# HuiGuanLab/DL-DKD

Hardware: NVIDIA B200
Metric: query-video pairs scored+ranked/sec (higher is better)
Workload: dtype bf16

## Files before the change

### dl-dkd_b200/_lib.py

```python
import ctypes
import os
from ctypes import c_char_p, c_float, c_int32, c_int64, c_void_p

_HERE = os.path.dirname(os.path.abspath(__file__))
LIB_PATH = os.path.join(_HERE, "libdkd_b200.so")

_P = c_void_p
_I = c_int32
_L = c_int64
_F = c_float

PROTOTYPES = {
    "dkd_version": [],
    "dkd_error_string": [_I],
    "dkd_normalize_rows": [_P, _L, _I, _F, _P, _P, _P, _L, _P],
    "dkd_downsample_clips": [_P, _P, _I, _I, _I, _I, _P, _P],
    "dkd_build_proposals": [_P, _I, _I, _I, _P, _P, _P, _P],
    "dkd_score_max_f32": [_P, _I, _P, _I, _I, _I, _P, _P, _P, _L, _P, _P, _P, _P],
    "dkd_row_planes_bytes": [_I, _I, _I],
    "dkd_pack_rows_tf32": [_P, _I, _I, _I, _P, _P],
    "dkd_score_max_exact": [_P, _I, _P, _I, _I, _I, _P, _P, _P, _L, _P, _P, _P],
    "dkd_clip_planes_bytes": [_I, _I],
    "dkd_pack_clips_tf32": [_P, _I, _I, _I, _P, _P],
    "dkd_clip_score_f32": [_P, _I, _P, _P, _I, _I, _I, _P, _P, _L, _P, _P, _P, _P, _P, _L, _P],
    "dkd_score_max_bf16": [_P, _I, _I, _P, _I, _I, _I, _P, _P, _P, _P, _L, _P, _F, _P],
    "dkd_score_max_f16": [_P, _I, _I, _P, _I, _I, _I, _P, _P, _P, _P, _L, _P, _F, _P],
    "dkd_score_max_bf16_lists": [_P, _I, _I, _P, _I, _I, _I, _P, _P, _P, _L, _F, _P, _P, _L, _I, _P],
    "dkd_clip_score_list": [_P, _I, _P, _P, _I, _I, _I, _P, _P, _L, _P, _P, _L, _P],
    "dkd_build_proposals_f16": [_P, _I, _I, _I, _P, _P, _P],
    "dkd_select_flagged": [_P, _I, _I, _L, _L, _P, _P, _P, _P, _P, _P],
    "dkd_select_pairs_csr": [_P, _I, _I, _L, _F, _L, _P, _P, _P, _P, _P],
    "dkd_key_clip_dots": [_P, _P, _I, _I, _I, _I, _P, _P],
    "dkd_frame_attn_table": [_P, _P, _P, _I, _I, _I, _I, _P, _P, _P],
    "dkd_frame_fuse": [_P, _P, _I, _P, _P, _I, _I, _I, _I, _L, _F, _F, _F, _I, _P, _P, _P],
    "dkd_fuse_scores": [_P, _P, _F, _F, _P, _L, _P],
    "dkd_topk": [_P, _I, _I, _L, _I, _I, _P, _P, _P],
    "dkd_select_topk": [_P, _I, _I, _L, _I, _I, _P, _P, _P],
    "dkd_merge_topk": [_P, _P, _I, _I, _I, _P, _P, _P],
    "dkd_rank_of_gt": [_P, _I, _I, _L, _P, _P, _P, _P],
    "dkd_candidates_to_csr": [_P, _I, _I, _I, _I, _P, _P, _P, _P, _P],
    "dkd_frame_fuse_csr": [_P, _P, _P, _P, _P, _P, _P, _I, _I, _I, _F, _F, _F, _I, _P, _L, _P],
    "dkd_scatter_fuse": [_P, _P, _F, _F, _P, _P, _I, _L, _P, _P],
    "dkd_sort_candidates": [_P, _P, _I, _I, _I, _P, _P, _P],
    "dkd_sort_candidates_payload": [_P, _P, _P, _I, _I, _I, _I, _P, _P, _P, _P],
    "dkd_merge_topk_payload": [_P, _P, _P, _I, _I, _I, _I, _P, _P, _P, _P],
    "dkd_frame_fuse_csr_detail": [_P, _P, _P, _P, _P, _P, _P, _I, _I, _I, _F, _F, _F, _I, _P, _L, _P, _I, _I, _P],
    "dkd_scatter_fuse_detail": [_P, _P, _F, _F, _P, _P, _P, _P, _I, _L, _P, _P, _I, _P],
    "dkd_weight_planes_bytes": [_I, _I],
    "dkd_pack_weight_tf32": [_P, _I, _I, _P, _P],
    "dkd_linear_exact": [_P, _L, _I, _P, _I, _P, _I, _P, _P, _L, _P],
    "dkd_row_stats": [_P, _L, _I, _F, _P, _P],
    "dkd_layernorm_rows": [_P, _L, _L, _I, _P, _P, _F, _P, _L, _P, _I, _P, _P],
    "dkd_mha_small": [_P, _L, _I, _I, _I, _P, _I, _I, _I, _I, _F, _P, _L, _P],
    "dkd_row_inv_norms": [_P, _L, _I, _F, _P, _P],
    "dkd_train_curve": [_P, _P, _P, _P, _I, _I, _I, _P, _P],
    "dkd_train_sim_fwd": [_P, _P, _P, _P, _P, _P, _I, _I, _I, _I, _P, _P, _P, _P, _P, _P],
    "dkd_train_sim_bwd": [_P, _P, _P, _P, _P, _P, _I, _I, _I, _I, _P, _P, _P, _P, _P, _P, _P, _P, _P, _P],
    "dkd_kl_curve_loss": [_P, _P, _P, _I, _I, _F, _P, _P, _P],
    "dkd_train_losses_workspace_floats": [_I, _I],
    "dkd_train_losses": [_P, _P, _P, _P, _P, _P, _I, _I, _F, _I, _F, _F, _P, _P, _P, _P, _P],
}
_RESTYPES = {"dkd_error_string": c_char_p, "dkd_clip_planes_bytes": c_int64, "dkd_row_planes_bytes": c_int64,
             "dkd_weight_planes_bytes": c_int64,
             "dkd_train_losses_workspace_floats": c_int64}

_lib = None


class DkdError(RuntimeError):
    pass


def load():
    global _lib
    if _lib is not None:
        return _lib
    if not os.path.exists(LIB_PATH):
        raise DkdError(
            f"{LIB_PATH} not found: build it with `python dl-dkd_b200/build.py` "
            "(nvcc, sm_100a). dkd_b200 has no CPU / PyTorch fallback for the scoring path.")
    lib = ctypes.CDLL(LIB_PATH)
    for name, argtypes in PROTOTYPES.items():
        fn = getattr(lib, name)
        fn.argtypes = argtypes
        fn.restype = _RESTYPES.get(name, c_int32)
    _lib = lib
    return lib


def check(code: int, what: str):
    if code != 0:
        msg = load().dkd_error_string(code)
        raise DkdError(f"{what} failed with code {code}: {msg.decode() if msg else '?'}")


KERNELS_PER_CALL = {"dkd_candidates_to_csr": 3, "dkd_select_pairs_csr": 3, "dkd_train_sim_bwd": 2, "dkd_train_losses": 3,
                    "dkd_train_losses_workspace_floats": 0}
_launches = 0
_timed_names = set()
_timed_events = {}


def reset_counters():
    global _launches
    _launches = 0


def launch_count() -> int:
    return _launches


def set_timed(names):
    global _timed_names, _timed_events
    _timed_names = set(names)
    _timed_events = {n: [] for n in _timed_names}


def timed_results():
    import torch
    torch.cuda.synchronize()
    return {n: [a.elapsed_time(b) for a, b in evs] for n, evs in _timed_events.items()}


def call(name: str, *args):
    global _launches
    lib = load()
    if name in _timed_names:
        import torch
        a, b = torch.cuda.Event(enable_timing=True), torch.cuda.Event(enable_timing=True)
        a.record()
        check(getattr(lib, name)(*args), name)
        b.record()
        _timed_events[name].append((a, b))
    else:
        check(getattr(lib, name)(*args), name)
    _launches += KERNELS_PER_CALL.get(name, 1)
```

### dl-dkd_b200/csrc/dkd_exact_umma.cu

```cuda
#include "dkd_umma.cuh"
#include "dkd_scan.cuh"

namespace dkd {

constexpr int kXRows = 128;
constexpr int kXKB = 32;
constexpr int kXScanWarps = 4;
constexpr int kXStageWarps = 8;
constexpr int kXStagers = 4 * 32;
constexpr int kXMmaWarp = kXScanWarps + kXStageWarps;
constexpr int kXLoadWarp = kXMmaWarp + 1;
constexpr int kXThreads = (kXLoadWarp + 1) * 32;
constexpr int kXMaxAStages = 7;
constexpr int kXBStages = 3;
constexpr uint32_t kXBPlane = 32 * 128;
constexpr int kXTmemCols = 512;
constexpr uint32_t kXRowPitch = 128;
constexpr uint32_t kXSlotBytes = 32 * kXRowPitch;
constexpr uint32_t kXScanScratch = 32 * kXRows * 4;

struct ExactParams {
  const float* q; int M;
  const float* planes; const float* scale;
  int Nv, T, D;
  int b_bufs;
  int R, Npad;
  const uint8_t* mask;
  float* out_max; int32_t* out_arg; int64_t ld_out;
  const int32_t* vid_ptr; const int32_t* vid_cnt; const int32_t* q_list; const int32_t* out_slot;
  unsigned wait_ns;
  int Nv_real, tile_chunks, tiles_per_chunk;
  int64_t list_stride;
  const int32_t* known_key;
  int64_t known_ld;
  const float2* row_ss;
  const float* bias;
  int relu, n_cols;
};
constexpr int kXGroup = 4;
#ifndef DKD_X_LIST_SCAN
#define DKD_X_LIST_SCAN 0
#endif
#ifndef DKD_X_KNOWN
#define DKD_X_KNOWN 1
#endif
#ifndef DKD_X_STREAM_B0
#define DKD_X_STREAM_B0 0
#endif
#ifndef DKD_X_RING0
#define DKD_X_RING0 5
#endif
constexpr bool kXStreamB0 = DKD_X_STREAM_B0 != 0;
constexpr int kXListScan = DKD_X_LIST_SCAN;
constexpr int kXKnown = DKD_X_KNOWN;
constexpr bool kXTwoPhaseList = kXListScan != 0 || kXKnown != 0;

struct __align__(8) ExactCtl {
  uint64_t a_full[kXMaxAStages], a_empty[kXMaxAStages];
  uint64_t b_full[kXBStages], b_empty[kXBStages];
  uint64_t tmem_full[2], tmem_empty[2];
  uint32_t tmem_base;
};

__device__ __forceinline__ void cp_async16(uint32_t dst, const void* src, uint32_t src_bytes) {
  asm volatile("cp.async.cg.shared.global [%0], [%1], 16, %2;" ::"r"(dst), "l"(src), "r"(src_bytes) : "memory");
}
__device__ __forceinline__ void cp_async_commit() { asm volatile("cp.async.commit_group;" ::: "memory"); }
template <int N>
__device__ __forceinline__ void cp_async_wait() { asm volatile("cp.async.wait_group %0;" ::"n"(N) : "memory"); }
__device__ __forceinline__ void bulk_load(void* dst, const void* src, uint32_t bytes, uint64_t* bar) {
  asm volatile("cp.async.bulk.shared::cluster.global.mbarrier::complete_tx::bytes [%0], [%1], %2, [%3];"
               ::"r"(smem_u32(dst)), "l"(src), "r"(bytes), "r"(smem_u32(bar)) : "memory");
}
__device__ __forceinline__ void fence_proxy_async() { asm volatile("fence.proxy.async.shared::cta;" ::: "memory"); }
__device__ __forceinline__ void split_tf32(float x, uint32_t& hi, uint32_t& lo) {
  hi = (__float_as_uint(x) + 0x1000u) & 0xffffe000u;
  lo = __float_as_uint(x - __uint_as_float(hi));
}

__device__ __forceinline__ void tmem_st_16x256b_x4(uint32_t taddr, const uint32_t* r) {
  asm volatile(
      "tcgen05.st.sync.aligned.16x256b.x4.b32 [%0], {%1,%2,%3,%4,%5,%6,%7,%8,%9,%10,%11,%12,%13,%14,%15,%16};"
      ::"r"(taddr), "r"(r[0]), "r"(r[1]), "r"(r[2]), "r"(r[3]), "r"(r[4]), "r"(r[5]), "r"(r[6]), "r"(r[7]),
        "r"(r[8]), "r"(r[9]), "r"(r[10]), "r"(r[11]), "r"(r[12]), "r"(r[13]), "r"(r[14]), "r"(r[15])
      : "memory");
}
__device__ __forceinline__ void tmem_st_wait() { asm volatile("tcgen05.wait::st.sync.aligned;" ::: "memory"); }

__device__ __forceinline__ void umma_tf32_ts(uint32_t tmem_d, uint32_t tmem_a, uint64_t bdesc, uint32_t idesc, uint32_t accum) {
  asm volatile(
      "{\n\t.reg .pred p;\n\t"
      "setp.ne.b32 p, %4, 0;\n\t"
      "tcgen05.mma.cta_group::1.kind::tf32 [%0], [%1], %2, %3, p;\n\t}"
      ::"r"(tmem_d), "r"(tmem_a), "l"(bdesc), "r"(idesc), "r"(accum)
      : "memory");
}
__host__ __device__ __forceinline__ uint32_t make_idesc_tf32(int n, int m) {
  return (1u << 4) | (2u << 7) | (2u << 10) | ((uint32_t)(n >> 3) << 17) | ((uint32_t)(m >> 4) << 24);
}

__device__ __forceinline__ uint32_t sw128_off(int r, int c) {
  return (uint32_t)((r >> 3) * 1024 + (r & 7) * 128 + ((c ^ (r & 7)) << 4));
}

__device__ __forceinline__ void video_range(const ExactParams& p, int n, int& e0, int& count) {
  if (p.vid_ptr) { e0 = p.vid_ptr[n]; count = p.vid_cnt ? p.vid_cnt[n] : p.vid_ptr[n + 1] - e0; }
  else if (p.list_stride > 0) {
    e0 = (int)((int64_t)n * p.list_stride);
    count = p.vid_cnt[n];
    if (count > (int)p.list_stride) count = (int)p.list_stride;
  }
  else { e0 = 0; count = p.M; }
}

__device__ __forceinline__ void item_range(const ExactParams& p, int item, int& group, int& row0, int& count) {
  group = item / p.tile_chunks;
  const int chunk = item - group * p.tile_chunks;
  row0 = chunk * p.tiles_per_chunk * kXRows;
  const int rows = p.tiles_per_chunk * kXRows;
  count = p.M - row0 < rows ? p.M - row0 : rows;
}

__device__ __forceinline__ void item_range_linear(const ExactParams& p, int item, int& wtile, int& row0, int& count) {
  wtile = item % p.Nv_real;
  const int chunk = item / p.Nv_real;
  row0 = chunk * p.tiles_per_chunk * kXRows;
  const int rows = p.tiles_per_chunk * kXRows;
  count = p.M - row0 < rows ? p.M - row0 : rows;
}

template <int kMode, bool kT32, int kXRing>
__global__ void __launch_bounds__(kXThreads, 1)
exact_umma_kernel(const ExactParams p) {
  constexpr int kDW = kMode == 0 ? 32 : 128;
  constexpr int kScaleBufs = kMode == 2 ? kXGroup : 2;
  constexpr int kStageSets = kMode == 2 ? 1 : 2;
  constexpr int kScanGroups = (kMode == 0 && kXTwoPhaseList) ? 1 : 0;
  constexpr bool kResB = kMode == 0 && !kXStreamB0;
  constexpr uint32_t kXACol0 = 2 * kDW;
  constexpr int kXStages = (kXTmemCols - 2 * kDW) / 64;
  extern __shared__ __align__(1024) uint8_t smem_raw_x[];
  __shared__ __align__(16) float s_scale[kScaleBufs][32 * 32];
  uint8_t* smem = reinterpret_cast<uint8_t*>((reinterpret_cast<uintptr_t>(smem_raw_x) + 1023) & ~(uintptr_t)1023);
  const int num_kb = p.D / kXKB;
  const uint32_t b_buf_bytes = kResB ? (uint32_t)num_kb * 2u * kXBPlane : 2u * (uint32_t)p.Npad * 128u;
  uint8_t* sB = smem;
  uint8_t* sS = sB + (size_t)(kResB ? p.b_bufs : kXBStages) * b_buf_bytes;
  float* sD = reinterpret_cast<float*>(sS + (size_t)(4 * kStageSets) * kXRing * kXSlotBytes);
  ExactCtl* ctl = reinterpret_cast<ExactCtl*>(reinterpret_cast<uint8_t*>(sD) + (size_t)kScanGroups * kXScanScratch);
  const int warp = threadIdx.x >> 5, lane = threadIdx.x & 31;
  const uint32_t b_bufs = (uint32_t)p.b_bufs;

  if (threadIdx.x == 0) {
    for (int i = 0; i < kXStages; ++i) { mbar_init(&ctl->a_full[i], kXStagers); mbar_init(&ctl->a_empty[i], 1); }
    for (int i = 0; i < kXBStages; ++i) { mbar_init(&ctl->b_full[i], 1); mbar_init(&ctl->b_empty[i], 1); }
    for (int i = 0; i < 2; ++i) {
      mbar_init(&ctl->tmem_full[i], 1);
      mbar_init(&ctl->tmem_empty[i], kXScanWarps);
    }
    fence_barrier_init();
  }
  if (warp == kXMmaWarp) {
    asm volatile("tcgen05.alloc.cta_group::1.sync.aligned.shared::cta.b32 [%0], %1;" ::"r"(smem_u32(&ctl->tmem_base)), "n"(kXTmemCols));
    asm volatile("tcgen05.relinquish_alloc_permit.cta_group::1.sync.aligned;");
  }
  tc_fence_before();
  __syncthreads();
  tc_fence_after();
  const uint32_t tmem_base = ctl->tmem_base;

  if (warp >= kXScanWarps && warp < kXScanWarps + 4 * kStageSets) {
    const int quarter = warp & 3, par = (warp - kXScanWarps) >> 2;
    const int g = lane >> 2, t = lane & 3;
    const int cl_row = lane >> 3, cl_chunk = lane & 7;
    const uint32_t a_lane = tmem_base + ((uint32_t)(quarter * 32) << 16) + kXACol0;
    const int sw = warp - kXScanWarps;
    const uint32_t ring0 = smem_u32(sS) + (uint32_t)sw * kXRing * kXSlotBytes;
    const uint8_t* ring_ptr = sS + (size_t)sw * kXRing * kXSlotBytes;
    uint32_t it_base = 0;
    for (int n = blockIdx.x; n < p.Nv; n += gridDim.x) {
      int e0, count, row_base = 0;
      if (kMode == 2) { int g_; item_range(p, n, g_, row_base, count); e0 = 0; }
      else if (kMode == 4) { int g_; item_range_linear(p, n, g_, row_base, count); e0 = 0; }
      else video_range(p, n, e0, count);
      if (count <= 0) continue;
      int ss_tile = -1;
      float2 ss[4];
      const int nitems = ((count + kXRows - 1) / kXRows) * num_kb;
      int t_cached = -1;
      const float* src_cached[8];
      uint32_t live_mask = 0;
      int iss_tile = 0, iss_kb = par;
      while (iss_kb >= num_kb) { iss_kb -= num_kb; ++iss_tile; }
      auto issue = [&](int slot) {
        const int tile = iss_tile, kb = iss_kb;
        iss_kb += kStageSets;
        while (iss_kb >= num_kb) { iss_kb -= num_kb; ++iss_tile; }
        if (tile != t_cached) {
          t_cached = tile;
          live_mask = 0;
#pragma unroll
          for (int i = 0; i < 8; ++i) {
            const int r = tile * kXRows + quarter * 32 + 4 * i + cl_row;
            const bool live = r < count;
            const int64_t qrow = live ? (p.q_list ? (int64_t)p.q_list[e0 + r] : (int64_t)(row_base + r)) : 0;
            src_cached[i] = p.q + qrow * p.D + 4 * cl_chunk;
            live_mask |= (live ? 1u : 0u) << i;
          }
        }
        const uint32_t dst = ring0 + (uint32_t)slot * kXSlotBytes + (uint32_t)cl_row * kXRowPitch +
                             (uint32_t)((cl_chunk ^ ((cl_row & 1) << 2)) << 4);
#pragma unroll
        for (int i = 0; i < 8; ++i)
          cp_async16(dst + (uint32_t)(4 * i) * kXRowPitch, src_cached[i] + kb * kXKB, ((live_mask >> i) & 1u) ? 16u : 0u);
      };
      auto store = [&](int j, int slot_i) {
        const uint8_t* slot = ring_ptr + (size_t)slot_i * kXSlotBytes;
        float4 v[8];
#pragma unroll
        for (int hu = 0; hu < 4; ++hu)
#pragma unroll
          for (int c = 0; c < 2; ++c)
            v[2 * hu + c] = *reinterpret_cast<const float4*>(
                slot + (16 * (hu >> 1) + g + 8 * (hu & 1)) * kXRowPitch + (((4 * c + t) ^ ((g & 1) << 2)) << 4));
        if (kMode == 4) {
          if (p.row_ss) {
            const int tile_j = j / num_kb;
            if (tile_j != ss_tile) {
              ss_tile = tile_j;
#pragma unroll
              for (int hu = 0; hu < 4; ++hu) {
                const int r = tile_j * kXRows + quarter * 32 + 16 * (hu >> 1) + g + 8 * (hu & 1);
                ss[hu] = r < count ? __ldg(p.row_ss + row_base + r) : make_float2(0.f, 0.f);
              }
            }
#pragma unroll
            for (int hu = 0; hu < 4; ++hu)
#pragma unroll
              for (int c = 0; c < 2; ++c) {
                float4& x = v[2 * hu + c];
                x.x = fmaf(x.x, ss[hu].x, ss[hu].y); x.y = fmaf(x.y, ss[hu].x, ss[hu].y);
                x.z = fmaf(x.z, ss[hu].x, ss[hu].y); x.w = fmaf(x.w, ss[hu].x, ss[hu].y);
              }
          }
        }
        const uint32_t it = it_base + (uint32_t)j;
        const uint32_t stage = it % (uint32_t)kXStages;
        const uint32_t phase = (it / (uint32_t)kXStages) & 1u;
        mbar_wait_backoff(&ctl->a_empty[stage], phase ^ 1u, 5 * p.wait_ns);
        tc_fence_after();
#pragma unroll
        for (int h = 0; h < 2; ++h) {
          uint32_t rh[16], rl[16];
#pragma unroll
          for (int u = 0; u < 2; ++u)
#pragma unroll
            for (int c = 0; c < 2; ++c) {
              const float4 x = v[2 * (2 * h + u) + c];
              split_tf32(x.x, rh[4 * (2 * c) + 2 * u + 0], rl[4 * (2 * c) + 2 * u + 0]);
              split_tf32(x.y, rh[4 * (2 * c) + 2 * u + 1], rl[4 * (2 * c) + 2 * u + 1]);
              split_tf32(x.z, rh[4 * (2 * c + 1) + 2 * u + 0], rl[4 * (2 * c + 1) + 2 * u + 0]);
              split_tf32(x.w, rh[4 * (2 * c + 1) + 2 * u + 1], rl[4 * (2 * c + 1) + 2 * u + 1]);
            }
          const uint32_t ta = a_lane + ((uint32_t)(16 * h) << 16) + stage * 64u;
          tmem_st_16x256b_x4(ta, rh);
          tmem_st_16x256b_x4(ta + 32u, rl);
        }
        tmem_st_wait();
        tc_fence_before();
        mbar_arrive(&ctl->a_full[stage]);
      };
      const int nmine = (nitems - par + kStageSets - 1) / kStageSets;
#pragma unroll
      for (int m = 0; m < kXRing - 1; ++m) {
        if (m < nmine) issue(m);
        cp_async_commit();
      }
      for (int m = 0; m < nmine; ++m) {
        if (m + kXRing - 1 < nmine) issue((m + kXRing - 1) % kXRing);
        cp_async_commit();
        cp_async_wait<kXRing - 1>();
        __syncwarp();
        store(kStageSets * m + par, m % kXRing);
        __syncwarp();
      }
      cp_async_wait<0>();
      it_base += (uint32_t)nitems;
    }
  } else if (warp == kXLoadWarp) {
    if (lane == 0) {
      uint32_t vi = 0, itb = 0;
      for (int n = blockIdx.x; n < p.Nv; n += gridDim.x) {
        int e0, count;
        if (kMode == 2) {
          int g_, row0_;
          item_range(p, n, g_, row0_, count);
          if (count <= 0) continue;
          const uint8_t* base = reinterpret_cast<const uint8_t*>(p.planes);
          for (int t0 = 0; t0 < count; t0 += kXRows) {
            for (int kb = 0; kb < num_kb; ++kb, ++itb) {
              const uint32_t bs = itb % (uint32_t)kXBStages;
              mbar_wait_backoff(&ctl->b_empty[bs], ((itb / (uint32_t)kXBStages) & 1u) ^ 1u, 5 * p.wait_ns);
              mbar_expect_tx(&ctl->b_full[bs], b_buf_bytes);
              for (int v = 0; v < kXGroup; ++v) {
                const int vid = min(g_ * kXGroup + v, p.Nv_real - 1);
                const uint8_t* src = base + ((size_t)vid * num_kb + kb) * 2 * kXBPlane;
                bulk_load(sB + (size_t)bs * b_buf_bytes + (size_t)v * kXBPlane, src, kXBPlane, &ctl->b_full[bs]);
                bulk_load(sB + (size_t)bs * b_buf_bytes + (size_t)(kXGroup + v) * kXBPlane, src + kXBPlane, kXBPlane,
                          &ctl->b_full[bs]);
              }
            }
          }
          continue;
        }
        int vid = n;
        if (kMode == 4) { int r0_; item_range_linear(p, n, vid, r0_, count); }
        else video_range(p, n, e0, count);
        if (count <= 0) continue;
        if (kResB) {
          const uint32_t bb = vi % b_bufs;
          mbar_wait_backoff(&ctl->b_empty[bb], ((vi / b_bufs) & 1u) ^ 1u, 5 * p.wait_ns);
          ++vi;
          mbar_expect_tx(&ctl->b_full[bb], b_buf_bytes);
          const uint8_t* src = reinterpret_cast<const uint8_t*>(p.planes) + (size_t)n * b_buf_bytes;
          for (int kb = 0; kb < num_kb; ++kb)
            bulk_load(sB + (size_t)bb * b_buf_bytes + (size_t)kb * 2 * kXBPlane, src + (size_t)kb * 2 * kXBPlane,
                      2 * kXBPlane, &ctl->b_full[bb]);
        } else {
          const uint8_t* src = reinterpret_cast<const uint8_t*>(p.planes) + (size_t)vid * num_kb * b_buf_bytes;
          for (int t0 = 0; t0 < count; t0 += kXRows) {
            for (int kb = 0; kb < num_kb; ++kb, ++itb) {
              const uint32_t bs = itb % (uint32_t)kXBStages;
              mbar_wait_backoff(&ctl->b_empty[bs], ((itb / (uint32_t)kXBStages) & 1u) ^ 1u, 5 * p.wait_ns);
              mbar_expect_tx(&ctl->b_full[bs], b_buf_bytes);
              bulk_load(sB + (size_t)bs * b_buf_bytes, src + (size_t)kb * b_buf_bytes, b_buf_bytes, &ctl->b_full[bs]);
            }
          }
        }
      }
    }
  } else if (warp == kXMmaWarp) {
    const int nb = kMode == 0 ? 32 : p.Npad;
    const uint32_t idesc = make_idesc_tf32(nb, kXRows);
    const uint32_t b_plane = (uint32_t)nb * 128u;
    const bool elected = elect_one();
    const uint64_t bdesc0 = make_smem_desc(smem_u32(sB));
    uint32_t it = 0, vi = 0, tc = 0, itb = 0;
    for (int n = blockIdx.x; n < p.Nv; n += gridDim.x) {
      int e0, count;
      if (kMode == 2) { int g_, r_; item_range(p, n, g_, r_, count); e0 = 0; }
      else if (kMode == 4) { int g_, r_; item_range_linear(p, n, g_, r_, count); e0 = 0; }
      else video_range(p, n, e0, count);
      if (count <= 0) continue;
      uint32_t bb = 0;
      if (kResB) {
        bb = vi % b_bufs;
        mbar_wait_backoff(&ctl->b_full[bb], (vi / b_bufs) & 1u, p.wait_ns);
        ++vi;
      }
      for (int t0 = 0; t0 < count; t0 += kXRows, ++tc) {
        const uint32_t buf = tc & 1u;
        mbar_wait_backoff(&ctl->tmem_empty[buf], ((tc >> 1) & 1u) ^ 1u, p.wait_ns);
        tc_fence_after();
        const uint32_t d_tmem = tmem_base + buf * (uint32_t)kDW;
        for (int kb = 0; kb < num_kb; ++kb, ++it) {
          const uint32_t stage = it % (uint32_t)kXStages;
          const uint32_t phase = (it / (uint32_t)kXStages) & 1u;
          uint32_t bs = 0;
          if (!kResB) {
            bs = itb % (uint32_t)kXBStages;
            mbar_wait_backoff(&ctl->b_full[bs], (itb / (uint32_t)kXBStages) & 1u, p.wait_ns);
            ++itb;
          }
          mbar_wait_backoff(&ctl->a_full[stage], phase, p.wait_ns);
          tc_fence_after();
          if (elected) {
            const uint32_t a_hi = tmem_base + kXACol0 + stage * 64u;
            const uint32_t a_lo = a_hi + 32u;
            const uint64_t b_hi = kResB ? bdesc0 + (uint64_t)((bb * b_buf_bytes + (uint32_t)kb * 2u * b_plane) >> 4)
                                             : bdesc0 + (uint64_t)((bs * b_buf_bytes) >> 4);
            const uint64_t b_lo = b_hi + (uint64_t)(b_plane >> 4);
#pragma unroll
            for (int k = 0; k < 4; ++k) {
              umma_tf32_ts(d_tmem, a_lo + 8 * k, b_hi + 2 * k, idesc, (kb | k) ? 1u : 0u);
              umma_tf32_ts(d_tmem, a_hi + 8 * k, b_lo + 2 * k, idesc, 1u);
              umma_tf32_ts(d_tmem, a_hi + 8 * k, b_hi + 2 * k, idesc, 1u);
            }
            umma_commit(&ctl->a_empty[stage]);
            if (!kResB) umma_commit(&ctl->b_empty[bs]);
          }
          __syncwarp();
        }
        if (elected) umma_commit(&ctl->tmem_full[buf]);
        __syncwarp();
      }
      if (kResB) {
        if (elected) umma_commit(&ctl->b_empty[bb]);
        __syncwarp();
      }
    }
  } else if constexpr (kMode == 2) {
    const int T = p.T, P = T * (T + 1) / 2;
    const int quarter = warp & 3;
    const uint32_t part = warp >= 2 * kXScanWarps ? 1u : 0u;
    const int stid = threadIdx.x;
    uint32_t tc = 0;
    for (int n = blockIdx.x; n < p.Nv; n += gridDim.x) {
      int group, row0, count;
      item_range(p, n, group, row0, count);
      if (count <= 0) continue;
      asm volatile("bar.sync 1, %0;" ::"n"(2 * kXScanWarps * 32) : "memory");
      if (part == 0) {
        for (int v = 0; v < kXGroup; ++v) {
          const int vid = min(group * kXGroup + v, p.Nv_real - 1);
          const float* gsc = p.scale + (int64_t)vid * P;
          const int s_ = stid & 31;
          int base = 0;
          for (int w = 1; w <= T; ++w) {
            if ((w & 3) == (stid >> 5) && s_ + w <= T) s_scale[v][(w - 1) * 32 + s_] = __ldg(gsc + base + s_);
            base += T - w + 1;
          }
        }
      }
      asm volatile("bar.sync 1, %0;" ::"n"(2 * kXScanWarps * 32) : "memory");
      for (int t0 = 0; t0 < count; t0 += kXRows, ++tc) {
        const uint32_t buf = tc & 1u;
        if (buf != part) continue;
        mbar_wait(&ctl->tmem_full[buf], (tc >> 1) & 1u);
        tc_fence_after();
        const int r = row0 + t0 + quarter * 32 + lane;
#pragma unroll 1
        for (int v = 0; v < kXGroup; ++v) {
          uint32_t raw[32];
          tmem_ld32_issue(tmem_base + ((uint32_t)(quarter * 32) << 16) + buf * (uint32_t)kDW + (uint32_t)(32 * v), raw);
          tmem_ld_wait();
          if (v == kXGroup - 1) {
            tc_fence_before();
            __syncwarp();
            if (lane == 0) mbar_arrive(&ctl->tmem_empty[buf]);
          }
          const float* sc = s_scale[v];
          float d[32];
#pragma unroll
          for (int i = 0; i < 32; ++i) d[i] = __uint_as_float(raw[i]);
          float bv0;
          int bi0;
          window_scan_v1<kT32>(d, sc, T, bv0, bi0);
          const int vid = group * kXGroup + v;
          if (r < p.M && t0 + quarter * 32 + lane < count && vid < p.Nv_real) {
            const int64_t o = (int64_t)r * p.ld_out + vid;
            p.out_max[o] = bv0;
            if (p.out_arg) p.out_arg[o] = bi0;
          }
        }
      }
    }
  } else if constexpr (kMode == 0) {
    const int T = p.T, P = T * (T + 1) / 2;
    const int quarter = warp;
    const int stid = threadIdx.x;
    uint32_t tc = 0, vi = 0;
    for (int n = blockIdx.x; n < p.Nv; n += gridDim.x) {
      int e0, count;
      video_range(p, n, e0, count);
      if (count <= 0) continue;
      float* sc = s_scale[vi & 1u];
      {
        const float* gsc = p.scale + (int64_t)n * P;
        const int s_ = stid & 31;
        int base = 0;
        for (int w = 1; w <= T; ++w) {
          if ((w & 3) == (stid >> 5) && s_ + w <= T) sc[(w - 1) * 32 + s_] = __ldg(gsc + base + s_);
          base += T - w + 1;
        }
      }
      asm volatile("bar.sync 1, %0;" ::"n"(kXScanWarps * 32) : "memory");
      ++vi;
      for (int t0 = 0; t0 < count; t0 += kXRows, ++tc) {
        const uint32_t buf = tc & 1u;
        mbar_wait(&ctl->tmem_full[buf], (tc >> 1) & 1u);
        tc_fence_after();
        uint32_t raw[32];
        tmem_ld32_issue(tmem_base + ((uint32_t)(quarter * 32) << 16) + buf * (uint32_t)kDW, raw);
        tmem_ld_wait();
        tc_fence_before();
        __syncwarp();
        if (lane == 0) mbar_arrive(&ctl->tmem_empty[buf]);
        float d[32];
#pragma unroll
        for (int i = 0; i < 32; ++i) d[i] = __uint_as_float(raw[i]);
        float bv0;
        int bi0;
        const int r = t0 + quarter * 32 + lane;
        if constexpr (kT32 && kXTwoPhaseList) {
          float* dcol = sD + quarter * 32 + lane;
          if (kXKnown != 0 && p.known_key) {
            const int qi = r < count ? (p.q_list ? p.q_list[e0 + r] : r) : 0;
            const int key = r < count ? __ldg(p.known_key + (int64_t)qi * p.known_ld + n) : 0;
            window_scan_known<kXKnown == 2>(d, sc, dcol, kXRows, key, bv0, bi0);
          } else if (kXListScan != 0) {
            window_scan_v2<kXListScan == 2>(d, sc, dcol, kXRows, bv0, bi0);
          } else {
            window_scan_v1<kT32>(d, sc, T, bv0, bi0);
          }
        } else {
          window_scan_v1<kT32>(d, sc, T, bv0, bi0);
        }
        if (r < count) {
          const int64_t o = p.out_slot ? (int64_t)p.out_slot[e0 + r]
                            : (p.list_stride > 0 ? (int64_t)p.q_list[e0 + r] * p.ld_out + n
                                                 : (p.vid_ptr ? (int64_t)(e0 + r) : (int64_t)r * p.ld_out + n));
          p.out_max[o] = bv0;
          if (p.out_arg) p.out_arg[o] = bi0;
        }
      }
    }
  } else if constexpr (kMode == 4) {
    const int quarter = warp;
    uint32_t tc = 0;
    for (int n = blockIdx.x; n < p.Nv; n += gridDim.x) {
      int wtile, row0, count;
      item_range_linear(p, n, wtile, row0, count);
      if (count <= 0) continue;
      for (int t0 = 0; t0 < count; t0 += kXRows, ++tc) {
        const uint32_t buf = tc & 1u;
        mbar_wait(&ctl->tmem_full[buf], (tc >> 1) & 1u);
        tc_fence_after();
        const int r = t0 + quarter * 32 + lane;
        const bool live = r < count;
        float* orow = p.out_max + (int64_t)(row0 + (live ? r : 0)) * p.ld_out;
#pragma unroll 1
        for (int c0 = 0; c0 < 128; c0 += 32) {
          uint32_t raw[32];
          tmem_ld32_issue(tmem_base + ((uint32_t)(quarter * 32) << 16) + buf * (uint32_t)kDW + (uint32_t)c0, raw);
          tmem_ld_wait();
          if (c0 == 96) {
            tc_fence_before();
            __syncwarp();
            if (lane == 0) mbar_arrive(&ctl->tmem_empty[buf]);
          }
#pragma unroll
          for (int j = 0; j < 32; j += 4) {
            const int col = wtile * 128 + c0 + j;
            if (live && col < p.n_cols) {
              float4 o = make_float4(__uint_as_float(raw[j]), __uint_as_float(raw[j + 1]), __uint_as_float(raw[j + 2]),
                                     __uint_as_float(raw[j + 3]));
              if (p.bias) {
                const float4 b = __ldg(reinterpret_cast<const float4*>(p.bias + col));
                o.x += b.x; o.y += b.y; o.z += b.z; o.w += b.w;
              }
              if (p.relu) { o.x = fmaxf(o.x, 0.f); o.y = fmaxf(o.y, 0.f); o.z = fmaxf(o.z, 0.f); o.w = fmaxf(o.w, 0.f); }
              *reinterpret_cast<float4*>(orow + col) = o;
            }
          }
        }
      }
    }
  } else {
    const int quarter = warp;
    uint32_t tc = 0;
    for (int n = blockIdx.x; n < p.Nv; n += gridDim.x) {
      int e0, count;
      video_range(p, n, e0, count);
      if (count <= 0) continue;
      const uint8_t* mrow = p.mask ? p.mask + (int64_t)n * p.R : nullptr;
      for (int t0 = 0; t0 < count; t0 += kXRows, ++tc) {
        const uint32_t buf = tc & 1u;
        mbar_wait(&ctl->tmem_full[buf], (tc >> 1) & 1u);
        tc_fence_after();
        float bv = -INFINITY;
        int bi = 0;
        for (int c0 = 0; c0 < p.R; c0 += 32) {
          uint32_t raw[32];
          tmem_ld32_issue(tmem_base + ((uint32_t)(quarter * 32) << 16) + buf * (uint32_t)kDW + (uint32_t)c0, raw);
          tmem_ld_wait();
#pragma unroll
          for (int j = 0; j < 32; ++j) {
            const int r = c0 + j;
            if (r < p.R) {
              float v = __uint_as_float(raw[j]);
              if (mrow && __ldg(mrow + r) == 0) v = DKD_MASKED_SCORE;
              if (v > bv) { bv = v; bi = r; }
            }
          }
        }
        tc_fence_before();
        __syncwarp();
        if (lane == 0) mbar_arrive(&ctl->tmem_empty[buf]);
        const int r = t0 + quarter * 32 + lane;
        if (r < count) {
          const int64_t o = p.out_slot ? (int64_t)p.out_slot[e0 + r]
                                       : (p.vid_ptr ? (int64_t)(e0 + r) : (int64_t)r * p.ld_out + n);
          p.out_max[o] = bv;
          if (p.out_arg) p.out_arg[o] = bi;
        }
      }
    }
  }

  tc_fence_before();
  __syncthreads();
  if (warp == kXMmaWarp) {
    tc_fence_after();
    asm volatile("tcgen05.dealloc.cta_group::1.sync.aligned.b32 %0, %1;" ::"r"(tmem_base), "n"(kXTmemCols));
  }
}

__global__ void pack_rows_tf32_kernel(const float* __restrict__ x, int R, int rpad, int D, float* __restrict__ planes,
                                      int64_t total_rows) {
  const int n = blockIdx.x;
  const int num_kb = D / kXKB;
  const uint32_t plane_bytes = (uint32_t)rpad * 128u;
  uint8_t* dst = reinterpret_cast<uint8_t*>(planes) + (size_t)n * num_kb * 2 * plane_bytes;
  for (int i = threadIdx.x; i < num_kb * rpad * 8; i += blockDim.x) {
    const int kb = i / (rpad * 8), rem = i - kb * rpad * 8;
    const int r = rem >> 3, c8 = rem & 7;
    float4 v = make_float4(0.f, 0.f, 0.f, 0.f);
    if (r < R && (int64_t)n * R + r < total_rows) v = *reinterpret_cast<const float4*>(x + ((int64_t)n * R + r) * D + kb * kXKB + c8 * 4);
    uint2 h0, l0, h1, l1;
    split_tf32(v.x, h0.x, l0.x); split_tf32(v.y, h0.y, l0.y); split_tf32(v.z, h1.x, l1.x); split_tf32(v.w, h1.y, l1.y);
    const int cc = c8 >> 2, tt = c8 & 3;
    const int p0 = 16 * cc + 2 * tt;
    uint8_t* row0 = dst + (size_t)(kb * 2) * plane_bytes;
    uint8_t* d0 = row0 + sw128_off(r, p0 >> 2) + (p0 & 3) * 4;
    uint8_t* d1 = row0 + sw128_off(r, (p0 + 8) >> 2) + (p0 & 3) * 4;
    *reinterpret_cast<uint2*>(d0) = h0;
    *reinterpret_cast<uint2*>(d1) = h1;
    *reinterpret_cast<uint2*>(d0 + plane_bytes) = l0;
    *reinterpret_cast<uint2*>(d1 + plane_bytes) = l1;
  }
}

}

using namespace dkd;

static int row_pad(int R, int clip_mode) { return clip_mode ? 32 : ((R + 15) / 16) * 16; }

extern "C" int64_t dkd_clip_planes_bytes(int32_t Nv, int32_t D) {
  if (Nv < 0 || D <= 0 || D % kXKB != 0) return -1;
  return (int64_t)Nv * (D / kXKB) * 2 * kXBPlane;
}
extern "C" int64_t dkd_row_planes_bytes(int32_t Nv, int32_t R, int32_t D) {
  if (Nv < 0 || R <= 0 || R > 128 || D <= 0 || D % kXKB != 0) return -1;
  return (int64_t)Nv * (D / kXKB) * 2 * row_pad(R, 0) * 128;
}

static int pack_rows(const float* x, int32_t Nv, int32_t R, int32_t rpad, int32_t D, float* planes, void* stream) {
  if (!x || !planes || Nv < 0) return DKD_ERR_ARG;
  if (R <= 0 || R > rpad || D <= 0 || D % kXKB != 0 || D > 512) return DKD_ERR_SHAPE;
  if ((reinterpret_cast<uintptr_t>(x) | reinterpret_cast<uintptr_t>(planes)) & 15) return DKD_ERR_ALIGN;
  if (Nv == 0) return DKD_OK;
  pack_rows_tf32_kernel<<<Nv, 256, 0, (cudaStream_t)stream>>>(x, R, rpad, D, planes, (int64_t)Nv * R);
  DKD_LAUNCH_CHECK();
  return DKD_OK;
}
extern "C" int dkd_pack_clips_tf32(const float* clips, int32_t Nv, int32_t T, int32_t D, float* planes, void* stream) {
  if (T > 32) return DKD_ERR_SHAPE;
  return pack_rows(clips, Nv, T, 32, D, planes, stream);
}
extern "C" int dkd_pack_rows_tf32(const float* xn, int32_t Nv, int32_t R, int32_t D, float* planes, void* stream) {
  if (R > 128) return DKD_ERR_SHAPE;
  return pack_rows(xn, Nv, R, row_pad(R, 0), D, planes, stream);
}

static int launch_exact(int mode, ExactParams p, int32_t D, int32_t T, cudaStream_t st) {
  p.wait_ns = 0u;
  int dev = 0, sms = 0, max_smem = 0;
  DKD_CUDA_TRY(cudaGetDevice(&dev));
  DKD_CUDA_TRY(cudaDeviceGetAttribute(&sms, cudaDevAttrMultiProcessorCount, dev));
  DKD_CUDA_TRY(cudaDeviceGetAttribute(&max_smem, cudaDevAttrMaxSharedMemoryPerBlockOptin, dev));
  const int num_kb = D / kXKB;
  const bool stream0 = mode == 0 && kXStreamB0;
  const int ring = stream0 ? DKD_X_RING0 : ((mode == 0 || mode == 2) && D > 448 ? 2 : 3);
  const int ring_warps = mode == 2 ? 4 : kXStageWarps;
  const int scan_groups = (mode == 0 && kXTwoPhaseList) ? 1 : 0;
  const size_t fixed = sizeof(ExactCtl) + 1024 + 128 + 16384  +
                       (size_t)ring_warps * ring * kXSlotBytes + (size_t)scan_groups * kXScanScratch;
  size_t b_total;
  if (mode == 0 && !stream0) {
    const size_t b_buf = (size_t)num_kb * 2 * kXBPlane;
    if ((size_t)max_smem < fixed + b_buf) return DKD_ERR_SHAPE;
    p.b_bufs = ((size_t)max_smem >= fixed + 2 * b_buf) ? 2 : 1;
    b_total = (size_t)p.b_bufs * b_buf;
  } else {
    p.b_bufs = kXBStages;
    b_total = (size_t)kXBStages * 2 * p.Npad * 128;
    if ((size_t)max_smem < fixed + b_total) return DKD_ERR_SHAPE;
  }
  const size_t smem = fixed - 16384 + b_total;
  const int grid = p.Nv < sms ? p.Nv : sms;
  auto launch = [&](auto kern) -> int {
    DKD_CUDA_TRY(cudaFuncSetAttribute(kern, cudaFuncAttributeMaxDynamicSharedMemorySize, (int)smem));
    kern<<<grid, kXThreads, smem, st>>>(p);
    return DKD_OK;
  };
  int rc;
  if (mode == 0 && stream0) {
    rc = (T == 32) ? launch(exact_umma_kernel<0, true, DKD_X_RING0>) : launch(exact_umma_kernel<0, false, DKD_X_RING0>);
  } else if (mode == 0) {
    if (ring == 3) rc = (T == 32) ? launch(exact_umma_kernel<0, true, 3>) : launch(exact_umma_kernel<0, false, 3>);
    else rc = (T == 32) ? launch(exact_umma_kernel<0, true, 2>) : launch(exact_umma_kernel<0, false, 2>);
  } else if (mode == 2) {
    if (ring == 3) rc = (T == 32) ? launch(exact_umma_kernel<2, true, 3>) : launch(exact_umma_kernel<2, false, 3>);
    else rc = (T == 32) ? launch(exact_umma_kernel<2, true, 2>) : launch(exact_umma_kernel<2, false, 2>);
  } else if (mode == 4) {
    rc = launch(exact_umma_kernel<4, true, 3>);
  } else {
    rc = launch(exact_umma_kernel<1, true, 3>);
  }
  if (rc) return rc;
  DKD_LAUNCH_CHECK();
  return DKD_OK;
}

extern "C" int dkd_score_max_exact(const float* qn, int32_t M, const float* row_planes, int32_t Nv, int32_t R,
                                   int32_t D, const uint8_t* mask, float* out_max, int32_t* out_arg,
                                   int64_t ld_out, const int32_t* vid_ptr, const int32_t* q_list, void* stream) {
  if (!qn || !row_planes || !out_max || M < 0 || Nv < 0) return DKD_ERR_ARG;
  if ((vid_ptr == nullptr) != (q_list == nullptr)) return DKD_ERR_ARG;
  if (R <= 0 || R > 128 || D <= 0 || D % kXKB != 0 || D > 512) return DKD_ERR_SHAPE;
  if (!vid_ptr && ld_out < Nv) return DKD_ERR_ARG;
  if ((reinterpret_cast<uintptr_t>(qn) | reinterpret_cast<uintptr_t>(row_planes)) & 15) return DKD_ERR_ALIGN;
  if (M == 0 || Nv == 0) return DKD_OK;
  ExactParams p{};
  p.q = qn; p.M = M; p.planes = row_planes; p.scale = nullptr;
  p.Nv = Nv; p.T = 0; p.D = D; p.R = R; p.Npad = row_pad(R, 0); p.mask = mask;
  p.out_max = out_max; p.out_arg = out_arg; p.ld_out = ld_out;
  p.vid_ptr = vid_ptr; p.vid_cnt = nullptr; p.q_list = q_list; p.out_slot = nullptr;
  return launch_exact(1, p, D, 0, (cudaStream_t)stream);
}

extern "C" int dkd_clip_score_f32(const float* qn, int32_t M, const float* clip_planes, const float* prop_scale,
                                  int32_t Nv, int32_t T, int32_t D, float* out_max, int32_t* out_arg,
                                  int64_t ld_out, const int32_t* vid_ptr, const int32_t* vid_cnt,
                                  const int32_t* q_list, const int32_t* out_slot, const int32_t* known_key,
                                  int64_t known_ld, void* stream) {
  if (!qn || !clip_planes || !prop_scale || !out_max || M < 0 || Nv < 0) return DKD_ERR_ARG;
  if ((vid_ptr == nullptr) != (q_list == nullptr)) return DKD_ERR_ARG;
  if ((out_slot || vid_cnt) && !vid_ptr) return DKD_ERR_ARG;
  if (known_key && (!vid_ptr || known_ld < Nv || T != 32)) return DKD_ERR_ARG;
  if (T <= 0 || T > 32 || D <= 0 || D % kXKB != 0 || D > 512) return DKD_ERR_SHAPE;
  if (!vid_ptr && ld_out < Nv) return DKD_ERR_ARG;
  if ((reinterpret_cast<uintptr_t>(qn) | reinterpret_cast<uintptr_t>(clip_planes) | reinterpret_cast<uintptr_t>(prop_scale)) & 15)
    return DKD_ERR_ALIGN;
  if (M == 0 || Nv == 0) return DKD_OK;
  ExactParams p{};
  p.q = qn; p.M = M; p.planes = clip_planes; p.scale = prop_scale;
  p.Nv = Nv; p.T = T; p.D = D; p.R = T; p.Npad = 32; p.mask = nullptr;
  p.out_max = out_max; p.out_arg = out_arg; p.ld_out = ld_out;
  p.vid_ptr = vid_ptr; p.vid_cnt = vid_cnt; p.q_list = q_list; p.out_slot = out_slot;
  p.known_key = known_key; p.known_ld = known_ld;
  if (!vid_ptr && Nv >= kXGroup) {
    const int groups = (Nv + kXGroup - 1) / kXGroup;
    const int tiles = (M + kXRows - 1) / kXRows;
    int sms = 148, dev = 0;
    if (cudaGetDevice(&dev) == cudaSuccess) cudaDeviceGetAttribute(&sms, cudaDevAttrMultiProcessorCount, dev);
    int chunks = 1;
    while (chunks < tiles && (int64_t)groups * chunks < (int64_t)sms * 12) ++chunks;
    p.tiles_per_chunk = (tiles + chunks - 1) / chunks;
    p.tile_chunks = (tiles + p.tiles_per_chunk - 1) / p.tiles_per_chunk;
    p.Nv_real = Nv;
    p.Nv = groups * p.tile_chunks;
    p.Npad = 128;
    return launch_exact(2, p, D, T, (cudaStream_t)stream);
  }
  return launch_exact(0, p, D, T, (cudaStream_t)stream);
}

extern "C" int64_t dkd_weight_planes_bytes(int32_t N, int32_t K) {
  if (N <= 0 || K <= 0 || K % kXKB != 0) return -1;
  return (int64_t)((N + 127) / 128) * (K / kXKB) * 2 * 128 * 128;
}

extern "C" int dkd_pack_weight_tf32(const float* w, int32_t N, int32_t K, float* planes, void* stream) {
  if (!w || !planes || N <= 0) return DKD_ERR_ARG;
  if (K <= 0 || K % kXKB != 0) return DKD_ERR_SHAPE;
  if ((reinterpret_cast<uintptr_t>(w) | reinterpret_cast<uintptr_t>(planes)) & 15) return DKD_ERR_ALIGN;
  pack_rows_tf32_kernel<<<(N + 127) / 128, 256, 0, (cudaStream_t)stream>>>(w, 128, 128, K, planes, (int64_t)N);
  DKD_LAUNCH_CHECK();
  return DKD_OK;
}

extern "C" int dkd_linear_exact(const float* x, int64_t M, int32_t K, const float* w_planes, int32_t N,
                                const float* bias, int32_t relu, const float* row_scale_shift, float* out,
                                int64_t ld_out, void* stream) {
  if (!x || !w_planes || !out || M < 0 || N <= 0) return DKD_ERR_ARG;
  if (K <= 0 || K % kXKB != 0 || N % 4 != 0 || ld_out < N || ld_out % 4 != 0 || M > 0x7fffff00LL) return DKD_ERR_SHAPE;
  if ((reinterpret_cast<uintptr_t>(x) | reinterpret_cast<uintptr_t>(w_planes) | reinterpret_cast<uintptr_t>(out) |
       reinterpret_cast<uintptr_t>(bias) | reinterpret_cast<uintptr_t>(row_scale_shift)) & 15)
    return DKD_ERR_ALIGN;
  if (M == 0) return DKD_OK;
  ExactParams p{};
  p.q = x; p.M = (int)M; p.planes = w_planes; p.scale = nullptr;
  p.T = 0; p.D = K; p.R = 128; p.Npad = 128; p.mask = nullptr;
  p.out_max = out; p.out_arg = nullptr; p.ld_out = ld_out;
  p.row_ss = reinterpret_cast<const float2*>(row_scale_shift); p.bias = bias; p.relu = relu; p.n_cols = N;
  const int wtiles = (N + 127) / 128;
  const int tiles = (int)((M + kXRows - 1) / kXRows);
  int sms = 148, dev = 0;
  if (cudaGetDevice(&dev) == cudaSuccess) cudaDeviceGetAttribute(&sms, cudaDevAttrMultiProcessorCount, dev);
  int chunks = 1;
  while (chunks < tiles && (int64_t)wtiles * chunks < (int64_t)sms * 6) ++chunks;
  p.tiles_per_chunk = (tiles + chunks - 1) / chunks;
  p.tile_chunks = (tiles + p.tiles_per_chunk - 1) / p.tiles_per_chunk;
  p.Nv_real = wtiles;
  p.Nv = wtiles * p.tile_chunks;
  return launch_exact(4, p, K, 0, (cudaStream_t)stream);
}

extern "C" int dkd_clip_score_list(const float* qn, int32_t M, const float* clip_planes, const float* prop_scale,
                                   int32_t Nv, int32_t T, int32_t D, float* out_max, int32_t* out_arg, int64_t ld_out,
                                   const int32_t* vid_cnt, const int32_t* q_list, int64_t list_stride, void* stream) {
  if (!qn || !clip_planes || !prop_scale || !out_max || !vid_cnt || !q_list || M < 0 || Nv < 0) return DKD_ERR_ARG;
  if (list_stride <= 0 || ld_out < Nv || (int64_t)Nv * list_stride > 0x7fffffffLL) return DKD_ERR_ARG;
  if (T <= 0 || T > 32 || D <= 0 || D % kXKB != 0 || D > 512) return DKD_ERR_SHAPE;
  if ((reinterpret_cast<uintptr_t>(qn) | reinterpret_cast<uintptr_t>(clip_planes) | reinterpret_cast<uintptr_t>(prop_scale)) & 15)
    return DKD_ERR_ALIGN;
  if (M == 0 || Nv == 0) return DKD_OK;
  ExactParams p{};
  p.q = qn; p.M = M; p.planes = clip_planes; p.scale = prop_scale;
  p.Nv = Nv; p.T = T; p.D = D; p.R = T; p.Npad = 32; p.mask = nullptr;
  p.out_max = out_max; p.out_arg = out_arg; p.ld_out = ld_out;
  p.vid_ptr = nullptr; p.vid_cnt = vid_cnt; p.q_list = q_list; p.out_slot = nullptr; p.list_stride = list_stride;
  return launch_exact(0, p, D, T, (cudaStream_t)stream);
}
```

### dl-dkd_b200/engine.py

```python
import math
from dataclasses import dataclass, field
from typing import List, Optional

import torch
import torch.nn.functional as F

from . import ops

BRANCH_WEIGHTS = (0.7, 0.3)


@dataclass
class BranchData:
    frames_n: Optional[torch.Tensor] = None
    frames_b: Optional[torch.Tensor] = None
    frame_planes: Optional[torch.Tensor] = None
    clips: Optional[torch.Tensor] = None
    clip_planes: Optional[torch.Tensor] = None
    prop_scale: Optional[torch.Tensor] = None
    prop_b: Optional[torch.Tensor] = None
    prop_h: Optional[torch.Tensor] = None
    frames_h: Optional[torch.Tensor] = None
    table_f: Optional[torch.Tensor] = None
    table_h: Optional[torch.Tensor] = None


@dataclass
class PreparedCorpus:
    Nv: int
    L: int
    D: int
    T: int
    id_base: int
    mask_u8: torch.Tensor
    lengths: torch.Tensor
    branches: List[BranchData] = field(default_factory=list)
    heads: tuple = ("frame", "two_scale")
    Lg: int = 0
    mask_g: Optional[torch.Tensor] = None
    Pg: int = 0
    prop_mask: Optional[torch.Tensor] = None

    @property
    def P(self):
        return ops.num_proposals(self.T)

    def nbytes(self):
        tot = 0
        for b in self.branches:
            for t in vars(b).values():
                if t is not None:
                    tot += t.numel() * t.element_size()
        return tot


def prepare_corpus(frames_by_branch, mask, attn_params=None, T=ops.T_CLIPS, heads=("frame", "two_scale"),
                   precisions=("exact", "bf16"), id_base=0) -> PreparedCorpus:
    f0 = frames_by_branch[0]
    Nv, L, D = f0.shape
    mask = mask.to(f0.device)
    mask_u8 = (mask > 0).to(torch.uint8).contiguous()
    lengths = mask_u8.sum(dim=1).to(torch.int32).contiguous()
    pc = PreparedCorpus(Nv=Nv, L=L, D=D, T=T, id_base=id_base, mask_u8=mask_u8, lengths=lengths, heads=tuple(heads))
    P = ops.num_proposals(T)
    pc.Lg, pc.Pg = ops.round_up(L, 16), ops.round_up(P, 16)
    pc.mask_g = mask_u8
    if pc.Lg != L:
        pc.mask_g = torch.zeros((Nv, pc.Lg), dtype=torch.uint8, device=f0.device)
        pc.mask_g[:, :L] = mask_u8
    if pc.Pg != P:
        pc.prop_mask = torch.zeros((Nv, pc.Pg), dtype=torch.uint8, device=f0.device)
        pc.prop_mask[:, :P] = 1
    if Nv == 0:
        pc.branches = [BranchData() for _ in frames_by_branch]
        return pc

    def pad_rows(t, R, Rg):
        if t is None or Rg == R:
            return t
        out = torch.zeros((Nv, Rg, D), dtype=t.dtype, device=t.device)
        out[:, :R] = t.view(Nv, R, D)
        return out.view(Nv * Rg, D)

    for bi, fr in enumerate(frames_by_branch):
        fr = fr.contiguous().float()
        bd = BranchData()
        if "frame" in heads:
            approx = "bf16" in precisions or "fp16" in precisions
            out = ops.normalize_rows(fr, want_f32="exact" in precisions or approx,
                                     want_bf16="bf16" in precisions, want_f16="fp16" in precisions)
            fn, fb, fh = out if len(out) == 3 else (out[0], out[1], None)
            bd.frames_n = None if fn is None else fn.view(Nv, L, D)
            bd.frames_b = pad_rows(fb, L, pc.Lg)
            bd.frames_h = pad_rows(fh, L, pc.Lg)
            if bd.frames_n is not None and D % 32 == 0:
                bd.frame_planes = ops.pack_rows(bd.frames_n)
        if "two_scale" in heads:
            if attn_params is None:
                raise ValueError("two_scale head needs the key/value projections (attn_params)")
            kw, kb, vw, vb = attn_params[bi]
            bd.clips = ops.downsample_clips(fr, lengths, T)
            bd.clip_planes = ops.pack_clips(bd.clips)
            pb, ps, _ = ops.build_proposals(bd.clips, want_bf16="bf16" in precisions, want_scale=True)
            bd.prop_b = None if pb is None else pad_rows(pb.view(-1, D), P, pc.Pg)
            bd.prop_scale = ps
            if "fp16" in precisions:
                bd.prop_h = pad_rows(ops.build_proposals_f16(bd.clips)[0].view(-1, D), P, pc.Pg)
            key = F.linear(fr, kw, kb).contiguous()
            val = F.linear(fr, vw, vb).contiguous()
            bd.table_f, bd.table_h = ops.frame_attn_table(key, val, bd.clips, lengths, want_f32=True,
                                                          want_f16=any(x in precisions for x in ("bf16", "fp16", "shortcut")))
            del key, val
        pc.branches.append(bd)
    return pc


@dataclass
class PreparedQueries:
    M: int
    Mpad: int
    qn: List[torch.Tensor]
    qb: List[torch.Tensor]
    qh: List[torch.Tensor]


_PAD_WORDS = {}


@dataclass
class HitDetail:
    arg: torch.Tensor
    score: torch.Tensor
    frame: Optional[torch.Tensor] = None

    @staticmethod
    def pad_words(nb, two_scale, device=None):
        key = (nb, bool(two_scale), str(device))
        if key not in _PAD_WORDS:
            ninf = torch.tensor([float("-inf")], dtype=torch.float32).view(torch.int32).item()
            _PAD_WORDS[key] = torch.tensor(([-1, ninf, ninf] if two_scale else [-1, ninf]) * nb, dtype=torch.int32,
                                           device=device)
        return _PAD_WORDS[key]

    @classmethod
    def padding(cls, M, K, nb, two_scale, device=None):
        return cls.unpack(cls.pad_words(nb, two_scale, device).expand(M, K, -1), nb, two_scale)

    def pack(self) -> torch.Tensor:
        M, K, nb = self.arg.shape
        parts = [self.arg, self.score.view(torch.int32)]
        if self.frame is not None:
            parts.append(self.frame.view(torch.int32))
        return torch.stack(parts, dim=-1).reshape(M, K, nb * len(parts))

    @classmethod
    def unpack(cls, words, nb, two_scale):
        M, K, _ = words.shape
        w = words.reshape(M, K, nb, 3 if two_scale else 2)
        return cls(arg=w[..., 0].contiguous(), score=w[..., 1].contiguous().view(torch.float32),
                   frame=w[..., 2].contiguous().view(torch.float32) if two_scale else None)

    @classmethod
    def cat(cls, details):
        return cls(arg=torch.cat([d.arg for d in details]), score=torch.cat([d.score for d in details]),
                   frame=None if details[0].frame is None else torch.cat([d.frame for d in details]))

    def patch(self, idx, other):
        self.arg[idx] = other.arg
        self.score[idx] = other.score
        if self.frame is not None:
            self.frame[idx] = other.frame


def _gather_detail(ids, id_base, args, scores, frames=None):
    valid = (ids >= 0).unsqueeze(-1)
    n = (ids.long() - id_base).clamp_(min=0)

    def take(mats, fill):
        out = torch.stack([m.gather(1, n) for m in mats], dim=-1)
        return out.masked_fill_(~valid, fill)

    return HitDetail(arg=take(args, -1), score=take(scores, float("-inf")),
                     frame=None if frames is None else take(frames, float("-inf")))


def prepare_queries(q_by_branch, want_bf16=True) -> PreparedQueries:
    M = q_by_branch[0].shape[0]
    Mpad = ops.round_up(max(M, 1), 256)
    qn, qb, qh = [], [], []
    if M == 0:
        return PreparedQueries(M=0, Mpad=Mpad, qn=[q.float() for q in q_by_branch], qb=[None] * len(q_by_branch),
                               qh=[None] * len(q_by_branch))
    for q in q_by_branch:
        f, b, h = ops.normalize_rows(q.contiguous().float(), want_f32=True, want_bf16=want_bf16, rows_pad=Mpad,
                                     want_f16=True)
        qn.append(f[:M])
        qb.append(b)
        qh.append(h)
    return PreparedQueries(M=M, Mpad=Mpad, qn=qn, qb=qb, qh=qh)


def _branch_weights(nb):
    return BRANCH_WEIGHTS[:nb] if nb == 2 else (1.0,)


def _exact_rows(bd: BranchData, qn, pc: PreparedCorpus, csr=None):
    if bd.frame_planes is not None:
        return ops.score_max_exact(qn, bd.frame_planes, pc.L, pc.mask_u8, csr=csr)
    s, a, _ = ops.score_max_f32(qn, bd.frames_n, pc.mask_u8, csr=csr)
    return s, a


def score_frame_head(pc: PreparedCorpus, pq: PreparedQueries, precision="exact", want_arg=False):
    out = []
    for bd, qn, qb, qh in zip(pc.branches, pq.qn, pq.qb, pq.qh):
        if precision == "exact":
            s, a = _exact_rows(bd, qn, pc)
        elif precision == "fp16":
            s, a = ops.score_max_bf16(qh, pq.M, bd.frames_h, pc.Nv, pc.Lg, pc.mask_g)
        else:
            s, a = ops.score_max_bf16(qb, pq.M, bd.frames_b, pc.Nv, pc.Lg, pc.mask_g)
        out.append((s, a))
    return out


AMBIGUITY_TAU = 1.0e-3
AMBIGUITY_TAU_F16 = AMBIGUITY_TAU / 8


def score_two_scale_head(pc: PreparedCorpus, pq: PreparedQueries, precision="exact", w_clip=0.7, w_frame=0.3,
                         want_frame=False, tau=None):
    nb = len(pc.branches)
    wbs = _branch_weights(nb)
    fused = None
    per = []
    if tau is None:
        tau = AMBIGUITY_TAU_F16 if precision == "fp16" else AMBIGUITY_TAU
    for bi, (bd, qn, qb, qh) in enumerate(zip(pc.branches, pq.qn, pq.qb, pq.qh)):
        if precision == "exact":
            s_clip, k_clip = ops.clip_score_f32(qn, bd.clip_planes, bd.prop_scale)
            q, tab = qn, bd.table_f
        elif precision == "shortcut":
            s_clip, k_clip = ops.clip_score_f32(qn, bd.clip_planes, bd.prop_scale)
            q, tab = qh, bd.table_h
        else:
            if precision == "fp16":
                qb, prop = qh, bd.prop_h
            else:
                prop = bd.prop_b
            if tau > 0:
                s_clip, k_clip, cnt, lst = ops.score_max_bf16_lists(qb, pq.M, prop, pc.Nv, pc.Pg, tau, mask=pc.prop_mask)
                ops.clip_score_list(qn, bd.clip_planes, bd.prop_scale, cnt, lst, s_clip, k_clip)
            else:
                s_clip, k_clip = ops.score_max_bf16(qb, pq.M, prop, pc.Nv, pc.Pg, mask=pc.prop_mask)
            q, tab = qh, bd.table_h
        wb = wbs[bi] if nb == 2 else 1.0
        fused, fr = ops.frame_fuse(q, tab, s_clip, k_clip, w_clip, w_frame, wb, fused=fused, accumulate=bi > 0,
                                   want_frame=want_frame)
        per.append(dict(clip=s_clip, key_clip=k_clip, frame=fr))
    return fused, per


CERT_EPS = 1.0e-3
CERT_EPS_F16 = 2.5e-4
STATS = {"certify_fallback_queries": 0, "certify_checked_queries": 0}


class PendingCertificate:

    def __init__(self, pc, pq, unsure, out_s, out_i, args, detail=None):
        self.pc, self.pq, self.unsure, self.out_s, self.out_i, self.args = pc, pq, unsure, out_s, out_i, args
        self.detail = detail
        self.host = torch.empty((1,), dtype=torch.int32).pin_memory()
        self.host.copy_(unsure.sum(dtype=torch.int32).reshape(1), non_blocking=True)
        self.event = torch.cuda.Event()
        self.event.record()

    def resolve(self):
        self.event.synchronize()
        return _apply_fallback(self.pc, self.pq, self.unsure, int(self.host[0]), self.out_s, self.out_i, self.args,
                               self.detail)


PENDING: List[PendingCertificate] = []


def finish(keep_last=0):
    n = 0
    while len(PENDING) > keep_last:
        n += PENDING.pop(0).resolve()
    return n


def poll():
    n = 0
    while PENDING and PENDING[0].event.query():
        n += PENDING.pop(0).resolve()
    return n


def _apply_fallback(pc, pq, unsure, n_unsure, out_s, out_i, args, detail=None):
    STATS["certify_checked_queries"] += pq.M
    STATS["certify_fallback_queries"] += n_unsure
    if n_unsure:
        nb = len(pc.branches)
        idx = unsure.nonzero().squeeze(1)
        sub = PreparedQueries(M=n_unsure, Mpad=ops.round_up(n_unsure, 256), qn=[q[idx].contiguous() for q in pq.qn],
                              qb=[None] * nb, qh=[None] * nb)
        if detail is None:
            es, ei = rank(pc, sub, precision="exact", **args)
        else:
            es, ei, ed = rank(pc, sub, precision="exact", return_detail=True, **args)
            detail.patch(idx, ed)
        out_s[idx] = es
        out_i[idx] = ei
    return n_unsure


def rank(pc: PreparedCorpus, pq: PreparedQueries, K=100, head="two_scale", precision="bf16", rescore=True,
         Kc=128, w_clip=0.7, w_frame=0.3, tau=None, certify=True, return_dense=False, return_detail=False):
    nb = len(pc.branches)
    wbs = _branch_weights(nb)
    two = head != "frame"
    if PENDING:
        poll()
    if pq.M == 0 or pc.Nv == 0:
        dev = pc.mask_u8.device
        out = (torch.full((pq.M, K), float("-inf"), dtype=torch.float32, device=dev),
               torch.full((pq.M, K), -1, dtype=torch.int32, device=dev))
        if return_dense:
            out += (torch.empty((pq.M, pc.Nv), dtype=torch.float32, device=dev),)
        return out + (HitDetail.padding(pq.M, K, nb, two, dev),) if return_detail else out
    dense_route = precision == "exact" or not rescore
    per = None
    if head == "frame":
        if precision == "shortcut":
            raise ValueError("precision='shortcut' is a two-scale variant (the frame head has no clip windows)")
        sc = score_frame_head(pc, pq, precision)
        fused = sc[0][0] if nb == 1 else ops.fuse_scores(sc[0][0], sc[1][0], wbs[0], wbs[1])
    else:
        fused, per = score_two_scale_head(pc, pq, precision, w_clip, w_frame, tau=tau,
                                          want_frame=return_detail and dense_route)
    extra = (fused,) if return_dense else ()
    if dense_route:
        out_s, out_i = ops.topk(fused, K, pc.id_base)
        if return_detail:
            if head == "frame":
                det = _gather_detail(out_i, pc.id_base, [a for _, a in sc], [s for s, _ in sc])
            else:
                det = _gather_detail(out_i, pc.id_base, [p["key_clip"] for p in per], [p["clip"] for p in per],
                                     [p["frame"] for p in per])
            extra += (det,)
        return (out_s, out_i) + extra
    Kc = max(Kc, K)
    cand, approx_kth = ops.select_topk(fused, Kc, pc.id_base)
    csr = ops.candidates_to_csr(cand, pc.Nv, pc.id_base)
    cand_scores = torch.full((pq.M, Kc), float("-inf"), dtype=torch.float32, device=cand.device)
    words = torch.empty((pq.M, Kc, nb * (3 if two else 2)), dtype=torch.int32, device=cand.device) if return_detail \
        else None
    if head == "frame":
        ex = [_exact_rows(bd, qn, pc, csr=csr[:2]) for bd, qn in zip(pc.branches, pq.qn)]
        if return_detail:
            b, ab = (ex[1][0], ex[1][1]) if nb == 2 else (None, None)
            ops.scatter_fuse_detail(ex[0][0], b, wbs[0], wbs[1] if nb == 2 else 0.0, ex[0][1], ab, csr, cand_scores,
                                    words)
        elif nb == 2:
            ops.scatter_fuse(ex[0][0], ex[1][0], wbs[0], wbs[1], csr, cand_scores)
        else:
            ops.scatter_fuse(ex[0][0], None, 1.0, 0.0, csr, cand_scores)
    else:
        for bi, (bd, qn) in enumerate(zip(pc.branches, pq.qn)):
            if precision == "shortcut":
                cs, ck = per[bi]["clip"], per[bi]["key_clip"]
            else:
                cs, ck = ops.clip_score_f32(qn, bd.clip_planes, bd.prop_scale, csr=csr[:2],
                                            known_key=per[bi]["key_clip"])
            wb = wbs[bi] if nb == 2 else 1.0
            if return_detail:
                ops.frame_fuse_csr_detail(qn, bd.table_f, cs, ck, csr, w_clip, w_frame, wb, cand_scores, bi > 0,
                                          words, 3 * bi)
            else:
                ops.frame_fuse_csr(qn, bd.table_f, cs, ck, csr, w_clip, w_frame, wb, cand_scores, bi > 0)
    detail = None
    if return_detail:
        out_s, out_i, out_w = ops.sort_candidates_payload(cand_scores, cand, words, K,
                                                          HitDetail.pad_words(nb, two, cand.device))
        detail = HitDetail.unpack(out_w, nb, two)
    else:
        out_s, out_i = ops.sort_candidates(cand_scores, cand, K)
    if certify and Kc < pc.Nv:
        unsure = out_s[:, K - 1] <= approx_kth + (CERT_EPS if precision == "bf16" else CERT_EPS_F16)
        args = dict(K=K, head=head, w_clip=w_clip, w_frame=w_frame)
        if certify == "deferred":
            PENDING.append(PendingCertificate(pc, pq, unsure, out_s, out_i, args, detail))
        else:
            _apply_fallback(pc, pq, unsure, int(unsure.sum()), out_s, out_i, args, detail)
    return (out_s, out_i) + extra + ((detail,) if return_detail else ())


def moment_frames(arg, ids, lengths, T=ops.T_CLIPS, head="two_scale"):
    valid = (ids >= 0).unsqueeze(-1) & (arg >= 0)
    if head == "frame":
        first, end = arg.long(), arg.long() + 1
    else:
        P = ops.num_proposals(T)
        ws = torch.tensor([ops.proposal_window(p, T) for p in range(P)], dtype=torch.long, device=arg.device)
        p = arg.long().clamp(0, P - 1)
        w, s = ws[p, 0], ws[p, 1]
        n = torch.as_tensor(lengths, device=arg.device)[ids.long().clamp(min=0)].unsqueeze(-1).expand_as(arg)
        nf, nl = n.float(), n.long()

        def a(i):
            return torch.minimum(torch.round(i.float() / T * nf).long(), nl - 1)

        first, end = a(s), torch.maximum(a(s + w), a(s + w - 1) + 1)
    out = torch.stack([first, end], dim=-1).to(torch.int32)
    return out.masked_fill_(~valid.unsqueeze(-1), -1)


def shard_range(Nv: int, rank_: int, world: int):
    per = (Nv + world - 1) // world
    lo = min(rank_ * per, Nv)
    return lo, min(lo + per, Nv)


def _merge_lists(scores, ids, words=None, pad=None):
    if words is None:
        return ops.merge_topk(scores, ids)
    return ops.merge_topk_payload(scores, ids, words, pad)


def merge_shards(local_scores, local_ids, group=None, merge_fn=None, exchange="query_block", gather=True, detail=None):
    import torch.distributed as dist
    world = dist.get_world_size(group)
    M, K = local_scores.shape
    if detail is None:
        merge = merge_fn or ops.merge_topk
        local = [local_scores.contiguous(), local_ids.contiguous()]
        finish = tuple
    else:
        nb, two = detail.arg.shape[-1], detail.frame is not None
        pad = HitDetail.pad_words(nb, two, local_scores.device)
        merge = merge_fn or (lambda s, i, w: _merge_lists(s, i, w, pad))
        local = [local_scores.contiguous(), local_ids.contiguous(), detail.pack()]

        def finish(res):
            return (res[0], res[1], HitDetail.unpack(res[2], nb, two))
    if world == 1:
        res = finish(local)
        return res if gather else res[:2] + ((0, M),) + res[2:]
    dev = local_scores.device
    nccl = dist.get_backend(group) == "nccl"
    if exchange == "all_gather":
        gathered = [torch.empty((world,) + t.shape, dtype=t.dtype, device=dev) for t in local]
        for g, t in zip(gathered, local):
            if nccl:
                dist.all_gather_into_tensor(g, t, group=group)
            else:
                dist.all_gather(list(g.unbind(0)), t, group=group)
        res = finish(merge(*gathered))
        return res if gather else res[:2] + ((0, M),) + res[2:]
    if exchange != "query_block":
        raise ValueError("exchange must be 'query_block' or 'all_gather'")
    rank_ = dist.get_rank(group)
    Mb = (M + world - 1) // world
    q_lo, q_hi = min(rank_ * Mb, M), min((rank_ + 1) * Mb, M)
    mine = q_hi - q_lo
    in_split = [min((g + 1) * Mb, M) - min(g * Mb, M) for g in range(world)]
    recv = [torch.empty((world, mine) + t.shape[1:], dtype=t.dtype, device=dev) for t in local]
    for r, t in zip(recv, local):
        row = math.prod(t.shape[1:])
        dist.all_to_all_single(r.view(world * mine, row), t.view(M, row), [mine] * world, in_split, group=group)
    if mine:
        block = list(merge(*recv))
    else:
        block = [r.new_empty((0,) + r.shape[2:]) for r in recv]
    if not gather:
        res = finish(block)
        return res[:2] + ((q_lo, q_hi),) + res[2:]
    if mine != Mb:
        fills = [float("-inf"), -1, -1]
        block = [torch.cat([b, b.new_full((Mb - mine,) + b.shape[1:], f)]) for b, f in zip(block, fills)]
    full = [torch.empty((world * Mb,) + b.shape[1:], dtype=b.dtype, device=dev) for b in block]
    for f, b in zip(full, block):
        if nccl:
            dist.all_gather_into_tensor(f, b.contiguous(), group=group)
        else:
            dist.all_gather(list(f.view((world, Mb) + b.shape[1:]).unbind(0)), b.contiguous(), group=group)
    return finish([f[:M] for f in full])


def split_queries(q_by_branch, batch=16384):
    Nq = q_by_branch[0].shape[0]
    return [prepare_queries([q[lo: lo + batch] for q in q_by_branch]) for lo in range(0, max(Nq, 1), batch)]


def iter_chunks(frames_by_branch, mask, chunk_videos=8192, id_base=0):
    Nv = frames_by_branch[0].shape[0]
    for lo in range(0, Nv, chunk_videos):
        hi = min(lo + chunk_videos, Nv)
        yield [f[lo:hi] for f in frames_by_branch], mask[lo:hi], id_base + lo


def rank_streamed(chunks, pqs, attn_params=None, K=100, T=ops.T_CLIPS, head="two_scale", precision="bf16",
                  rescore=True, Kc=128, w_clip=0.7, w_frame=0.3, tau=None, return_detail=False):
    running = [None] * len(pqs)
    precisions = ("exact", precision) if precision != "exact" else ("exact",)
    for frames, mask, id_base in chunks:
        pc = prepare_corpus(frames, mask, attn_params, T=T, heads=(head,), precisions=precisions, id_base=id_base)
        for b, pq in enumerate(pqs):
            out = rank(pc, pq, K=K, head=head, precision=precision, rescore=rescore, Kc=Kc, w_clip=w_clip,
                       w_frame=w_frame, tau=tau, return_detail=return_detail)
            if running[b] is None:
                running[b] = out
            elif not return_detail:
                running[b] = ops.merge_topk(torch.stack([running[b][0], out[0]]), torch.stack([running[b][1], out[1]]))
            else:
                d = out[2]
                s, i, w = _merge_lists(torch.stack([running[b][0], out[0]]), torch.stack([running[b][1], out[1]]),
                                       torch.stack([running[b][2].pack(), d.pack()]),
                                       HitDetail.pad_words(d.arg.shape[-1], d.frame is not None, d.arg.device))
                running[b] = (s, i, HitDetail.unpack(w, d.arg.shape[-1], d.frame is not None))
        del pc
    if any(r is None for r in running):
        raise ValueError("rank_streamed: the corpus has no chunks")
    res = (torch.cat([r[0] for r in running]), torch.cat([r[1] for r in running]))
    return res + (HitDetail.cat([r[2] for r in running]),) if return_detail else res
```

### dl-dkd_b200/eval.py

```python
import logging

import numpy as np
import torch
from torch.utils.data import DataLoader

from . import engine, ops

logger = logging.getLogger(__name__)


def _opt(opt, key, default):
    try:
        return getattr(opt, key)
    except AttributeError:
        if isinstance(opt, dict) and key in opt:
            return opt[key]
        return default


def _pad_stack(seqs):
    lens = [len(s) for s in seqs]
    out = torch.zeros(len(seqs), max(lens), seqs[0].shape[-1])
    mask = torch.zeros(len(seqs), max(lens))
    for i, s in enumerate(seqs):
        out[i, : lens[i]] = s[: lens[i]]
        mask[i, : lens[i]] = 1.0
    return out, mask


def collate_frame_val(data):
    if len(data[0]) == 3:
        feats, idxs, ids = zip(*data)
        videos, mask = _pad_stack(feats)
        return videos, mask, idxs, ids
    feats, teacher, idxs, ids = zip(*data)
    videos, mask = _pad_stack(feats)
    teacher_videos, _ = _pad_stack(teacher)
    return videos, teacher_videos, mask, idxs, ids


def collate_text_val(data):
    data = sorted(data, key=lambda x: len(x[0]), reverse=True)
    if len(data[0]) == 3:
        feats, idxs, ids = zip(*data)
        target, mask = _pad_stack(feats)
        return target, mask, idxs, ids
    feats, teacher, idxs, ids = zip(*data)
    target, mask = _pad_stack(feats)
    return target, torch.cat([t.reshape(1, -1) for t in teacher], dim=0), mask, idxs, ids


def _cat_padded(tensors):
    if not tensors:
        return None
    Lmax = max(t.shape[1] for t in tensors)
    n = sum(t.shape[0] for t in tensors)
    out = tensors[0].new_zeros((n, Lmax) + tuple(tensors[0].shape[2:]))
    if tensors[0].dim() not in (2, 3):
        raise ValueError("Only support 2/3 dimensional tensors")
    r = 0
    for t in tensors:
        out[r: r + t.shape[0], : t.shape[1]] = t
        r += t.shape[0]
    return out


def compute_context_info(model, eval_dataset, opt):
    model.eval()
    loader = DataLoader(eval_dataset, collate_fn=collate_frame_val, batch_size=opt.eval_context_bsz,
                        num_workers=_opt(opt, "num_workers", 0), shuffle=False, pin_memory=_opt(opt, "pin_memory", False))
    metas, inher, explore, teacher, masks = [], [], [], [], []
    with torch.no_grad():
        for batch in loader:
            metas.extend(batch[-1])
            feat = batch[0].to(opt.device, non_blocking=True)
            mask = batch[-3].to(opt.device, non_blocking=True)
            if len(batch) == 5:
                teacher.append(batch[1].to(opt.device, non_blocking=True))
            fi, fe = model.encode_context(feat, mask)
            inher.append(fi)
            explore.append(fe)
            masks.append(mask)
        inher = _cat_padded(inher)
        video_mask = _cat_padded(masks)
        explore = _cat_padded(explore) if model.double_branch else None
        scoring = _opt(opt, "scoring", "frame")
        precision = _opt(opt, "precision", "exact")
        prepared = model.prepare_context(inher, explore, video_mask, heads=(scoring,),
                                         precisions=("exact",) if precision == "exact" else ("exact", precision),
                                         id_base=_opt(opt, "id_base", 0))
    return dict(video_metas=metas, inher_frame_feat=inher, explore_frame_feat=explore,
                teacher_frame_feat=_cat_padded(teacher), video_mask=video_mask, prepared=prepared)


def _encode_all_queries(model, eval_dataset, opt):
    loader = DataLoader(eval_dataset, collate_fn=collate_text_val, batch_size=opt.eval_query_bsz,
                        num_workers=_opt(opt, "num_workers", 0), shuffle=False, pin_memory=_opt(opt, "pin_memory", False))
    metas, qi, qe, qt = [], [], [], []
    with torch.no_grad():
        for batch in loader:
            metas.extend(batch[-1])
            a, b = model.encode_query(batch[0].to(opt.device, non_blocking=True), batch[-3].to(opt.device, non_blocking=True))
            qi.append(a)
            qe.append(b)
            if len(batch) == 5:
                qt.append(batch[1].to(opt.device, non_blocking=True))
    qs = [torch.cat(qi, dim=0)]
    if model.double_branch:
        qs.append(torch.cat(qe, dim=0))
    return qs, metas, (torch.cat(qt, dim=0) if qt else None)


_PRECISIONS = ("exact", "bf16", "fp16", "shortcut")


def compute_query2ctx_info(model, eval_dataset, opt, ctx_info):
    model.eval()
    pc = ctx_info["prepared"]
    qs, metas, qt = _encode_all_queries(model, eval_dataset, opt)
    precision = _opt(opt, "precision", "exact")
    scoring = _opt(opt, "scoring", "frame")
    if precision not in _PRECISIONS:
        raise ValueError(f"opt.precision must be one of {_PRECISIONS}, got {precision!r}")
    chunk = int(_opt(opt, "query_chunk", 16384))
    outs = [[] for _ in qs]
    for lo in range(0, qs[0].shape[0], chunk):
        pq = engine.prepare_queries([q[lo: lo + chunk] for q in qs], want_bf16=precision == "bf16")
        if scoring == "frame":
            for o, (s, _) in zip(outs, engine.score_frame_head(pc, pq, precision)):
                o.append(s)
        else:
            for bi in range(len(qs)):
                sub = engine.PreparedCorpus(Nv=pc.Nv, L=pc.L, D=pc.D, T=pc.T, id_base=pc.id_base, mask_u8=pc.mask_u8,
                                            lengths=pc.lengths, branches=[pc.branches[bi]], heads=pc.heads,
                                            Lg=pc.Lg, mask_g=pc.mask_g, Pg=pc.Pg, prop_mask=pc.prop_mask)
                subq = engine.PreparedQueries(M=pq.M, Mpad=pq.Mpad, qn=[pq.qn[bi]], qb=[pq.qb[bi]], qh=[pq.qh[bi]])
                f, _ = engine.score_two_scale_head(sub, subq, precision, model.clip_scale_w, model.frame_scale_w)
                outs[bi].append(f)
    inher = torch.cat(outs[0], dim=0).cpu().numpy().copy()
    explore = torch.cat(outs[1], dim=0).cpu().numpy().copy() if model.double_branch else None
    teacher = None
    if ctx_info.get("teacher_frame_feat") is not None and qt is not None:
        teacher = model.get_sim_scores(qt, ctx_info["teacher_frame_feat"], ctx_info["video_mask"],
                                       want_rows=False)[0].cpu().numpy().copy()
    return inher, explore, teacher, metas


def rank_queries(model, eval_dataset, opt, ctx_info, K=100, return_dense=False, return_detail=False):
    model.eval()
    pc = ctx_info["prepared"]
    qs, metas, _ = _encode_all_queries(model, eval_dataset, opt)
    precision = _opt(opt, "precision", "exact")
    scoring = _opt(opt, "scoring", "frame")
    if precision not in _PRECISIONS:
        raise ValueError(f"opt.precision must be one of {_PRECISIONS}, got {precision!r}")
    chunk = int(_opt(opt, "query_chunk", 16384))
    outs = []
    for lo in range(0, qs[0].shape[0], chunk):
        pq = engine.prepare_queries([q[lo: lo + chunk] for q in qs], want_bf16=precision == "bf16")
        outs.append(engine.rank(pc, pq, K=K, head=scoring, precision=precision, w_clip=model.clip_scale_w,
                                w_frame=model.frame_scale_w, certify="deferred", return_dense=return_dense,
                                tau=_opt(opt, "ambiguity_tau", None), Kc=int(_opt(opt, "candidates", 128)),
                                return_detail=return_detail))
    engine.finish()
    res = tuple(engine.HitDetail.cat([o[j] for o in outs]) if isinstance(outs[0][j], engine.HitDetail)
                else torch.cat([o[j] for o in outs]) for j in range(len(outs[0])))
    return res[:2] + (metas,) + res[2:]


def get_gt(video_metas, query_metas):
    pos = {v: i for i, v in enumerate(video_metas)}
    v2t_gt = [[] for _ in video_metas]
    for i, qid in enumerate(query_metas):
        v = pos.get(qid.split('#', 1)[0])
        if v is not None:
            v2t_gt[v].append(i)
    t2v_gt = {}
    for v, qs in enumerate(v2t_gt):
        for q in qs:
            t2v_gt.setdefault(q, []).append(v)
    return v2t_gt, t2v_gt


def _gt_csr(q2m_gts, n_q, first_only=False):
    ptr = np.zeros(n_q + 1, np.int32)
    ids = []
    for i in range(n_q):
        g = list(q2m_gts[i])
        ids += g[:1] if first_only else g
        ptr[i + 1] = len(ids)
    return torch.from_numpy(ptr), torch.tensor(ids, dtype=torch.int32)


def gt_ranks(scores, q2m_gts, first_only=False, device="cuda"):
    s = torch.as_tensor(scores, dtype=torch.float32, device=device)
    zero = torch.zeros_like(s)
    sim = ops.fuse_scores(s.contiguous(), zero, -1.0, 0.0)
    ptr, ids = _gt_csr(q2m_gts, s.shape[0], first_only)
    return ops.rank_of_gt(sim, ptr.to(device), ids.to(device)).cpu().numpy()


def eval_q2m(scores, q2m_gts):
    r = gt_ranks(scores, q2m_gts)
    n_q = len(r)
    rk = [100.0 * np.count_nonzero(r <= k) / n_q for k in (1, 5, 10, 100)]
    return (rk[0], rk[1], rk[2], rk[3], np.median(r), r.mean())


def t2v_map(c2i, t2v_gts):
    r = gt_ranks(c2i, t2v_gts, first_only=True)
    return float(np.mean(1.0 / r))


def cal_perf(t2v_all_errors, t2v_gt, test=False):
    r1, r5, r10, r100, medr, meanr = eval_q2m(t2v_all_errors, t2v_gt)
    m = t2v_map(t2v_all_errors, t2v_gt)
    logger.info(" * Text to Video:")
    logger.info(" * r_1_5_10_100: {}".format([round(r1, 1), round(r5, 1), round(r10, 1), round(r100, 1)]))
    logger.info(" * recall sum: {}".format(round(r1 + r5 + r10 + r100, 1)))
    logger.info(" * mAP: {}".format(round(m, 4)))
    return (r1, r5, r10, r100, medr, meanr, m)


def recall_from_topk(top_ids, t2v_gt, ks=(1, 5, 10, 100)):
    ids = top_ids.cpu().numpy() if isinstance(top_ids, torch.Tensor) else np.asarray(top_ids)
    n_q = ids.shape[0]
    out = []
    for k in ks:
        hit = sum(1 for i in range(n_q) if set(t2v_gt.get(i, ())) & set(ids[i, :k].tolist()))
        out.append(100.0 * hit / n_q)
    return tuple(out)


def metrics_from_ranking(top_ids, dense, t2v_gt, id_base=0):
    M, K = top_ids.shape
    dev = top_ids.device
    ptr, gts = _gt_csr(t2v_gt, M)
    ptr1, first = _gt_csr(t2v_gt, M, first_only=True)
    ptr, gts, ptr1, first = ptr.to(dev), gts.to(dev), ptr1.to(dev), first.to(dev)

    def ranks(p, g):
        r_dense = ops.rank_of_gt(dense, p, g).long()
        cnt = (p[1:] - p[:-1]).long()
        owner = torch.repeat_interleave(torch.arange(M, device=dev), cnt)
        hit = top_ids[owner].long() == (g.long() + id_base).unsqueeze(1)
        pos = torch.where(hit.any(1), hit.float().argmax(1) + 1, torch.full_like(owner, K + 1))
        best = torch.full((M,), K + 1, dtype=torch.long, device=dev).scatter_reduce(0, owner, pos, "amin")
        return torch.where(best <= K, best, torch.maximum(r_dense, torch.full_like(r_dense, K + 1))).cpu().numpy()

    r = ranks(ptr, gts)
    rk = [100.0 * np.count_nonzero(r <= k) / M for k in (1, 5, 10, 100)]
    r1 = ranks(ptr1, first)
    return (rk[0], rk[1], rk[2], rk[3], np.median(r), r.mean(), float(np.mean(1.0 / r1)))


def _log_perf(m):
    logger.info(" * Text to Video:")
    logger.info(" * r_1_5_10_100: {}".format([round(x, 1) for x in m[:4]]))
    logger.info(" * recall sum: {}".format(round(sum(m[:4]), 1)))
    logger.info(" * mAP: {}".format(round(m[6], 4)))


def eval_epoch(model, val_video_dataset, val_text_dataset, opt, test=False):
    model.eval()
    precision = _opt(opt, "precision", "exact")
    if precision == "exact":
        with torch.no_grad():
            ctx = compute_context_info(model, val_video_dataset, opt)
            inher, explore, _, query_metas = compute_query2ctx_info(model, val_text_dataset, opt, ctx)
        _, t2v_gt = get_gt(ctx["video_metas"], query_metas)
        if _opt(opt, "double_branch", model.double_branch) and explore is not None:
            cal_perf(-1 * inher, t2v_gt, test)
            cal_perf(-1 * explore, t2v_gt, test)
            a = torch.from_numpy(inher).to(opt.device)
            b = torch.from_numpy(explore).to(opt.device)
            fused = ops.fuse_scores(a, b, 0.7, 0.3).cpu().numpy()
            r = cal_perf(-1 * fused, t2v_gt, test)
        else:
            r = cal_perf(-1 * inher, t2v_gt, test)
        return r[0] + r[1] + r[2] + r[3]
    with torch.no_grad():
        ctx = compute_context_info(model, val_video_dataset, opt)
        _, top_ids, query_metas, dense = rank_queries(model, val_text_dataset, opt, ctx, K=100, return_dense=True)
    _, t2v_gt = get_gt(ctx["video_metas"], query_metas)
    pc = ctx["prepared"]
    if _opt(opt, "per_branch_metrics", False) and model.double_branch:
        qs, _, _ = _encode_all_queries(model, val_text_dataset, opt)
        for bi in range(2):
            sub = engine.PreparedCorpus(Nv=pc.Nv, L=pc.L, D=pc.D, T=pc.T, id_base=pc.id_base, mask_u8=pc.mask_u8,
                                        lengths=pc.lengths, branches=[pc.branches[bi]], heads=pc.heads,
                                        Lg=pc.Lg, mask_g=pc.mask_g, Pg=pc.Pg, prop_mask=pc.prop_mask)
            pq = engine.prepare_queries([qs[bi]], want_bf16=precision == "bf16")
            _, ids_b, dense_b = engine.rank(sub, pq, K=100, head=_opt(opt, "scoring", "frame"), precision=precision,
                                            w_clip=model.clip_scale_w, w_frame=model.frame_scale_w, return_dense=True)
            _log_perf(metrics_from_ranking(ids_b, dense_b, t2v_gt, pc.id_base))
    m = metrics_from_ranking(top_ids, dense, t2v_gt, pc.id_base)
    _log_perf(m)
    return m[0] + m[1] + m[2] + m[3]
```

### dl-dkd_b200/ops.py

```python
import torch

from . import _lib

T_CLIPS = 32


def num_proposals(T: int = T_CLIPS) -> int:
    return T * (T + 1) // 2


def proposal_index(w: int, s: int, T: int = T_CLIPS) -> int:
    return (w - 1) * T - ((w - 1) * (w - 2)) // 2 + s


def proposal_window(p: int, T: int = T_CLIPS):
    if not 0 <= p < num_proposals(T):
        raise ValueError(f"proposal {p} out of range for T = {T}")
    w = 1
    while p >= T - w + 1:
        p -= T - w + 1
        w += 1
    return w, p


def _stream():
    return torch.cuda.current_stream().cuda_stream


def _p(t):
    return None if t is None else t.data_ptr()


def _chk(t, dtype, name):
    if not isinstance(t, torch.Tensor) or not t.is_cuda:
        raise _lib.DkdError(f"{name}: expected a CUDA tensor (dkd_b200 has no CPU path)")
    if t.dtype != dtype:
        raise _lib.DkdError(f"{name}: expected dtype {dtype}, got {t.dtype}")
    if not t.is_contiguous():
        raise _lib.DkdError(f"{name}: expected a contiguous tensor")
    return t


def round_up(x: int, m: int) -> int:
    return (x + m - 1) // m * m


def normalize_rows(x, want_f32=True, want_bf16=False, rows_pad=None, eps=1e-12, want_f16=False):
    _chk(x, torch.float32, "x")
    D = x.shape[-1]
    rows = x.numel() // D
    rows_pad = rows if rows_pad is None else rows_pad
    of = torch.empty((rows_pad, D), dtype=torch.float32, device=x.device) if want_f32 else None
    ob = torch.empty((rows_pad, D), dtype=torch.bfloat16, device=x.device) if want_bf16 else None
    oh = torch.empty((rows_pad, D), dtype=torch.float16, device=x.device) if want_f16 else None
    _lib.call("dkd_normalize_rows", _p(x), rows, D, eps, _p(of), _p(ob), _p(oh), rows_pad, _stream())
    return (of, ob, oh) if want_f16 else (of, ob)


def downsample_clips(frames, lengths, T=T_CLIPS):
    _chk(frames, torch.float32, "frames")
    _chk(lengths, torch.int32, "lengths")
    Nv, L, D = frames.shape
    clips = torch.empty((Nv, T, D), dtype=torch.float32, device=frames.device)
    _lib.call("dkd_downsample_clips", _p(frames), _p(lengths), Nv, L, D, T, _p(clips), _stream())
    return clips


def build_proposals_f16(clips, want_scale=False):
    _chk(clips, torch.float32, "clips")
    Nv, T, D = clips.shape
    P = num_proposals(T)
    ph = torch.empty((Nv, P, D), dtype=torch.float16, device=clips.device)
    ps = torch.empty((Nv, P), dtype=torch.float32, device=clips.device) if want_scale else None
    _lib.call("dkd_build_proposals_f16", _p(clips), Nv, T, D, _p(ph), _p(ps), _stream())
    return ph, ps


def build_proposals(clips, want_bf16=True, want_scale=True, want_f32=False):
    _chk(clips, torch.float32, "clips")
    Nv, T, D = clips.shape
    P = num_proposals(T)
    dev = clips.device
    pb = torch.empty((Nv, P, D), dtype=torch.bfloat16, device=dev) if want_bf16 else None
    ps = torch.empty((Nv, P), dtype=torch.float32, device=dev) if want_scale else None
    pf = torch.empty((Nv, P, D), dtype=torch.float32, device=dev) if want_f32 else None
    _lib.call("dkd_build_proposals", _p(clips), Nv, T, D, _p(pb), _p(ps), _p(pf), _stream())
    return pb, ps, pf


def score_max_f32(qn, xn, mask=None, want_rows=False, csr=None):
    _chk(qn, torch.float32, "qn")
    _chk(xn, torch.float32, "xn")
    M, D = qn.shape
    Nv, R, _ = xn.shape
    dev = qn.device
    if mask is not None:
        _chk(mask, torch.uint8, "mask")
    rows = torch.empty((M, R, Nv), dtype=torch.float32, device=dev) if want_rows else None
    if csr is None:
        om = torch.empty((M, Nv), dtype=torch.float32, device=dev)
        oa = torch.empty((M, Nv), dtype=torch.int32, device=dev)
        _lib.call("dkd_score_max_f32", _p(qn), M, _p(xn), Nv, R, D, _p(mask), _p(om), _p(oa), Nv, _p(rows),
                  None, None, _stream())
    else:
        vid_ptr, q_list = csr
        E = q_list.numel()
        om = torch.empty((E,), dtype=torch.float32, device=dev)
        oa = torch.empty((E,), dtype=torch.int32, device=dev)
        _lib.call("dkd_score_max_f32", _p(qn), M, _p(xn), Nv, R, D, _p(mask), _p(om), _p(oa), 0, _p(rows),
                  _p(vid_ptr), _p(q_list), _stream())
    return om, oa, rows


def pack_rows(xn):
    _chk(xn, torch.float32, "xn")
    Nv, R, D = xn.shape
    if D % 32 or R > 128:
        raise _lib.DkdError("pack_rows: D must be a multiple of 32 and R <= 128")
    planes = torch.empty((Nv, D // 32, 2, round_up(R, 16), 32), dtype=torch.float32, device=xn.device)
    _lib.call("dkd_pack_rows_tf32", _p(xn), Nv, R, D, _p(planes), _stream())
    return planes


def score_max_exact(qn, planes, R, mask=None, csr=None):
    _chk(qn, torch.float32, "qn")
    _chk(planes, torch.float32, "row_planes")
    M, D = qn.shape
    Nv = planes.shape[0]
    if planes.dim() != 5 or planes.shape[1] * 32 != D or planes.shape[3] != round_up(R, 16):
        raise _lib.DkdError("score_max_exact: row planes do not match (R, D)")
    if mask is not None:
        _chk(mask, torch.uint8, "mask")
    dev = qn.device
    if csr is None:
        om = torch.empty((M, Nv), dtype=torch.float32, device=dev)
        oa = torch.empty((M, Nv), dtype=torch.int32, device=dev)
        _lib.call("dkd_score_max_exact", _p(qn), M, _p(planes), Nv, R, D, _p(mask), _p(om), _p(oa), Nv, None, None,
                  _stream())
    else:
        vid_ptr, q_list = csr
        E = q_list.numel()
        om = torch.empty((E,), dtype=torch.float32, device=dev)
        oa = torch.empty((E,), dtype=torch.int32, device=dev)
        _lib.call("dkd_score_max_exact", _p(qn), M, _p(planes), Nv, R, D, _p(mask), _p(om), _p(oa), 0, _p(vid_ptr),
                  _p(q_list), _stream())
    return om, oa


def pack_clips(clips):
    _chk(clips, torch.float32, "clips")
    Nv, T, D = clips.shape
    if D % 32:
        raise _lib.DkdError("pack_clips: D must be a multiple of 32")
    planes = torch.empty((Nv, D // 32, 2, 32, 32), dtype=torch.float32, device=clips.device)
    _lib.call("dkd_pack_clips_tf32", _p(clips), Nv, T, D, _p(planes), _stream())
    return planes


def clip_score_f32(qn, clips, prop_scale, csr=None, scatter=None, known_key=None):
    _chk(qn, torch.float32, "qn")
    _chk(prop_scale, torch.float32, "prop_scale")
    planes = clips if clips.dim() == 5 else pack_clips(clips)
    _chk(planes, torch.float32, "clip_planes")
    M, D = qn.shape
    Nv, P = prop_scale.shape
    T = int(round(((8 * P + 1) ** 0.5 - 1) / 2))
    if planes.shape[0] != Nv or planes.shape[1] * 32 != D or T * (T + 1) // 2 != P:
        raise _lib.DkdError("clip_score_f32: clip planes / prop_scale / query shapes do not agree")
    dev = qn.device
    if csr is None:
        om = torch.empty((M, Nv), dtype=torch.float32, device=dev)
        oa = torch.empty((M, Nv), dtype=torch.int32, device=dev)
        _lib.call("dkd_clip_score_f32", _p(qn), M, _p(planes), _p(prop_scale), Nv, T, D, _p(om), _p(oa), Nv,
                  None, None, None, None, None, 0, _stream())
        return om, oa
    vid_ptr, q_list = csr[0], csr[1]
    vid_cnt = csr[2] if len(csr) > 2 else None
    if scatter is not None:
        slot, om, oa = scatter
        _chk(om, torch.float32, "out_max")
        _chk(oa, torch.int32, "out_arg")
    else:
        slot = None
        E = q_list.numel()
        om = torch.empty((E,), dtype=torch.float32, device=dev)
        oa = torch.empty((E,), dtype=torch.int32, device=dev)
    if known_key is not None:
        _chk(known_key, torch.int32, "known_key")
        if T != 32 or known_key.shape != (M, Nv):
            known_key = None
    _lib.call("dkd_clip_score_f32", _p(qn), M, _p(planes), _p(prop_scale), Nv, T, D, _p(om), _p(oa), 0,
              _p(vid_ptr), _p(vid_cnt), _p(q_list), _p(slot), _p(known_key), Nv if known_key is not None else 0, _stream())
    return om, oa


def score_max_bf16(q_bf16, M, x_bf16, Nv, R, mask=None, out_max=None, out_arg=None, want_gap=False, flag_tau=None):
    half = isinstance(q_bf16, torch.Tensor) and q_bf16.dtype == torch.float16
    _chk(q_bf16, torch.float16 if half else torch.bfloat16, "q_bf16")
    _chk(x_bf16, torch.float16 if half else torch.bfloat16, "x_bf16")
    Mpad, D = q_bf16.shape
    if x_bf16.numel() != Nv * R * D:
        raise _lib.DkdError("x_bf16 does not hold Nv*R rows of D features")
    if mask is not None:
        _chk(mask, torch.uint8, "mask")
    dev = q_bf16.device
    om = out_max if out_max is not None else torch.empty((M, Nv), dtype=torch.float32, device=dev)
    oa = out_arg if out_arg is not None else torch.empty((M, Nv), dtype=torch.int32, device=dev)
    og = torch.empty((M, Nv), dtype=torch.float32, device=dev) if want_gap else None
    fl = torch.zeros((M, (Nv + 31) // 32), dtype=torch.int32, device=dev) if flag_tau is not None else None
    _lib.call("dkd_score_max_f16" if half else "dkd_score_max_bf16", _p(q_bf16), M, Mpad, _p(x_bf16), Nv, R, D,
              _p(mask), _p(om), _p(oa), _p(og), Nv,
              _p(fl), float(flag_tau or 0.0), _stream())
    out = (om, oa)
    if want_gap:
        out += (og,)
    if flag_tau is not None:
        out += (fl,)
    return out


def score_max_bf16_lists(q, M, x, Nv, R, tau, mask=None):
    half = q.dtype == torch.float16
    _chk(q, torch.float16 if half else torch.bfloat16, "q")
    _chk(x, torch.float16 if half else torch.bfloat16, "x")
    Mpad, D = q.shape
    if x.numel() != Nv * R * D:
        raise _lib.DkdError("x does not hold Nv*R rows of D features")
    if mask is not None:
        _chk(mask, torch.uint8, "mask")
    dev = q.device
    om = torch.empty((M, Nv), dtype=torch.float32, device=dev)
    oa = torch.empty((M, Nv), dtype=torch.int32, device=dev)
    cnt = torch.zeros((Nv,), dtype=torch.int32, device=dev)
    lst = torch.empty((Nv, M), dtype=torch.int32, device=dev)
    _lib.call("dkd_score_max_bf16_lists", _p(q), M, Mpad, _p(x), Nv, R, D, _p(mask), _p(om), _p(oa), Nv, float(tau),
              _p(cnt), _p(lst), M, int(half), _stream())
    return om, oa, cnt, lst


def clip_score_list(qn, planes, prop_scale, cnt, lst, out_max, out_arg):
    _chk(qn, torch.float32, "qn")
    _chk(planes, torch.float32, "clip_planes")
    _chk(prop_scale, torch.float32, "prop_scale")
    _chk(cnt, torch.int32, "flag_cnt")
    _chk(lst, torch.int32, "flag_list")
    _chk(out_max, torch.float32, "out_max")
    _chk(out_arg, torch.int32, "out_arg")
    M, D = qn.shape
    Nv, P = prop_scale.shape
    T = int(round(((8 * P + 1) ** 0.5 - 1) / 2))
    _lib.call("dkd_clip_score_list", _p(qn), M, _p(planes), _p(prop_scale), Nv, T, D, _p(out_max), _p(out_arg),
              out_max.shape[1], _p(cnt), _p(lst), lst.shape[1], _stream())
    return out_max, out_arg


def select_flagged(flags, Nv, cap=None):
    _chk(flags, torch.int32, "flags")
    M = flags.shape[0]
    cap = M * Nv if cap is None else cap
    dev = flags.device
    cursor = torch.empty((1,), dtype=torch.int32, device=dev)
    vid_begin = torch.empty((Nv,), dtype=torch.int32, device=dev)
    vid_cnt = torch.empty((Nv,), dtype=torch.int32, device=dev)
    q_list = torch.empty((cap,), dtype=torch.int32, device=dev)
    slot = torch.empty((cap,), dtype=torch.int32, device=dev)
    _lib.call("dkd_select_flagged", _p(flags), M, Nv, Nv, cap, _p(cursor), _p(vid_begin), _p(vid_cnt), _p(q_list),
              _p(slot), _stream())
    return vid_begin, q_list, vid_cnt, slot


def select_pairs_csr(gap, tau, cap=None):
    _chk(gap, torch.float32, "gap")
    M, Nv = gap.shape
    cap = M * Nv if cap is None else cap
    dev = gap.device
    counts = torch.empty((Nv,), dtype=torch.int32, device=dev)
    vid_ptr = torch.empty((Nv + 1,), dtype=torch.int32, device=dev)
    q_list = torch.empty((cap,), dtype=torch.int32, device=dev)
    slot = torch.empty((cap,), dtype=torch.int32, device=dev)
    _lib.call("dkd_select_pairs_csr", _p(gap), M, Nv, Nv, tau, cap, _p(counts), _p(vid_ptr), _p(q_list), _p(slot),
              _stream())
    return vid_ptr, q_list, slot


def frame_attn_table(key, val, clips, lengths, want_f32=True, want_f16=True):
    _chk(key, torch.float32, "key")
    _chk(val, torch.float32, "val")
    _chk(clips, torch.float32, "clips")
    _chk(lengths, torch.int32, "lengths")
    Nv, L, D = key.shape
    T = clips.shape[1]
    P = num_proposals(T)
    dev = key.device
    E = torch.empty((Nv, L, T), dtype=torch.float32, device=dev)
    _lib.call("dkd_key_clip_dots", _p(key), _p(clips), Nv, L, T, D, _p(E), _stream())
    tf = torch.empty((Nv, P, D), dtype=torch.float32, device=dev) if want_f32 else None
    tb = torch.empty((Nv, P, D), dtype=torch.float16, device=dev) if want_f16 else None
    _lib.call("dkd_frame_attn_table", _p(E), _p(val), _p(lengths), Nv, L, T, D, _p(tf), _p(tb), _stream())
    return tf, tb


def frame_fuse(q, table, clip_scores, key_clip, w_clip, w_frame, w_branch, fused=None, accumulate=False,
               want_frame=False):
    is_f16 = q.dtype == torch.float16
    _chk(q, torch.float16 if is_f16 else torch.float32, "q")
    _chk(table, q.dtype, "table")
    _chk(key_clip, torch.int32, "key_clip")
    _chk(clip_scores, torch.float32, "clip_scores")
    M, Nv = key_clip.shape
    _, P, D = table.shape
    dev = key_clip.device
    fr = torch.empty((M, Nv), dtype=torch.float32, device=dev) if want_frame else None
    if fused is None:
        fused = torch.empty((M, Nv), dtype=torch.float32, device=dev)
        accumulate = False
    _lib.call("dkd_frame_fuse", _p(q), _p(table), int(is_f16), _p(clip_scores), _p(key_clip), M, Nv, P, D, Nv,
              w_clip, w_frame, w_branch, int(accumulate), _p(fr), _p(fused), _stream())
    return fused, fr


def fuse_scores(a, b, wa=0.7, wb=0.3):
    _chk(a, torch.float32, "a")
    _chk(b, torch.float32, "b")
    out = torch.empty_like(a)
    _lib.call("dkd_fuse_scores", _p(a), _p(b), wa, wb, _p(out), a.numel(), _stream())
    return out


def topk(scores, K, id_base=0):
    _chk(scores, torch.float32, "scores")
    M, Nv = scores.shape
    os_ = torch.empty((M, K), dtype=torch.float32, device=scores.device)
    oi = torch.empty((M, K), dtype=torch.int32, device=scores.device)
    _lib.call("dkd_topk", _p(scores), M, Nv, Nv, K, id_base, _p(os_), _p(oi), _stream())
    return os_, oi


def select_topk(scores, K, id_base=0):
    _chk(scores, torch.float32, "scores")
    M, Nv = scores.shape
    oi = torch.empty((M, K), dtype=torch.int32, device=scores.device)
    kth = torch.empty((M,), dtype=torch.float32, device=scores.device)
    _lib.call("dkd_select_topk", _p(scores), M, Nv, Nv, K, id_base, _p(oi), _p(kth), _stream())
    return oi, kth


def merge_topk(scores, ids):
    _chk(scores, torch.float32, "scores")
    _chk(ids, torch.int32, "ids")
    G, M, K = scores.shape
    os_ = torch.empty((M, K), dtype=torch.float32, device=scores.device)
    oi = torch.empty((M, K), dtype=torch.int32, device=scores.device)
    _lib.call("dkd_merge_topk", _p(scores), _p(ids), G, M, K, _p(os_), _p(oi), _stream())
    return os_, oi


def merge_topk_payload(scores, ids, payload, pad):
    _chk(scores, torch.float32, "scores")
    _chk(ids, torch.int32, "ids")
    _chk(payload, torch.int32, "payload")
    G, M, K = scores.shape
    C = payload.shape[-1]
    if payload.shape != (G, M, K, C) or pad.shape != (C,):
        raise _lib.DkdError("merge_topk_payload: payload must be (G, M, K, C) and pad (C,)")
    dev = scores.device
    os_ = torch.empty((M, K), dtype=torch.float32, device=dev)
    oi = torch.empty((M, K), dtype=torch.int32, device=dev)
    op = pad.to(device=dev, dtype=torch.int32).expand(M, K, C).contiguous()
    _lib.call("dkd_merge_topk_payload", _p(scores), _p(ids), _p(payload), G, M, K, C, _p(os_), _p(oi), _p(op), _stream())
    return os_, oi, op


def rank_of_gt(scores, gt_ptr, gt_ids):
    _chk(scores, torch.float32, "scores")
    _chk(gt_ptr, torch.int32, "gt_ptr")
    _chk(gt_ids, torch.int32, "gt_ids")
    M, Nv = scores.shape
    out = torch.empty((M,), dtype=torch.int32, device=scores.device)
    _lib.call("dkd_rank_of_gt", _p(scores), M, Nv, Nv, _p(gt_ptr), _p(gt_ids), _p(out), _stream())
    return out


def candidates_to_csr(cand_ids, Nv, id_base=0):
    _chk(cand_ids, torch.int32, "cand_ids")
    M, K = cand_ids.shape
    dev = cand_ids.device
    counts = torch.empty((Nv,), dtype=torch.int32, device=dev)
    vid_ptr = torch.empty((Nv + 1,), dtype=torch.int32, device=dev)
    q_list = torch.zeros((M * K,), dtype=torch.int32, device=dev)
    slot = torch.zeros((M * K,), dtype=torch.int32, device=dev)
    _lib.call("dkd_candidates_to_csr", _p(cand_ids), M, K, Nv, id_base, _p(counts), _p(vid_ptr), _p(q_list),
              _p(slot), _stream())
    return vid_ptr, q_list, slot


def frame_fuse_csr(q, table, clip_scores, key_clip, csr, w_clip, w_frame, w_branch, cand_scores, accumulate):
    _chk(q, torch.float32, "q")
    _chk(table, torch.float32, "table")
    _chk(clip_scores, torch.float32, "clip_scores")
    _chk(key_clip, torch.int32, "key_clip")
    vid_ptr, q_list, slot = csr
    Nv, P, D = table.shape
    dense_ld = clip_scores.shape[1] if clip_scores.dim() == 2 else 0
    _lib.call("dkd_frame_fuse_csr", _p(q), _p(table), _p(clip_scores), _p(key_clip), _p(vid_ptr), _p(q_list),
              _p(slot), Nv, P, D, w_clip, w_frame, w_branch, int(accumulate), _p(cand_scores), dense_ld, _stream())
    return cand_scores


def sort_candidates(cand_scores, cand_ids, K_out):
    _chk(cand_scores, torch.float32, "cand_scores")
    _chk(cand_ids, torch.int32, "cand_ids")
    M, K = cand_ids.shape
    os_ = torch.empty((M, K_out), dtype=torch.float32, device=cand_ids.device)
    oi = torch.empty((M, K_out), dtype=torch.int32, device=cand_ids.device)
    _lib.call("dkd_sort_candidates", _p(cand_scores), _p(cand_ids), M, K, K_out, _p(os_), _p(oi), _stream())
    return os_, oi


def sort_candidates_payload(cand_scores, cand_ids, payload, K_out, pad):
    _chk(cand_scores, torch.float32, "cand_scores")
    _chk(cand_ids, torch.int32, "cand_ids")
    _chk(payload, torch.int32, "payload")
    M, K = cand_ids.shape
    C = payload.shape[-1]
    if payload.shape != (M, K, C) or pad.shape != (C,):
        raise _lib.DkdError("sort_candidates_payload: payload must be (M, K, C) and pad (C,)")
    dev = cand_ids.device
    os_ = torch.empty((M, K_out), dtype=torch.float32, device=dev)
    oi = torch.empty((M, K_out), dtype=torch.int32, device=dev)
    op = pad.to(device=dev, dtype=torch.int32).expand(M, K_out, C).contiguous()
    _lib.call("dkd_sort_candidates_payload", _p(cand_scores), _p(cand_ids), _p(payload), M, K, K_out, C, _p(os_),
              _p(oi), _p(op), _stream())
    return os_, oi, op


def frame_fuse_csr_detail(q, table, clip_scores, key_clip, csr, w_clip, w_frame, w_branch, cand_scores, accumulate,
                          payload, c0):
    _chk(q, torch.float32, "q")
    _chk(table, torch.float32, "table")
    _chk(clip_scores, torch.float32, "clip_scores")
    _chk(key_clip, torch.int32, "key_clip")
    _chk(payload, torch.int32, "payload")
    vid_ptr, q_list, slot = csr
    Nv, P, D = table.shape
    dense_ld = clip_scores.shape[1] if clip_scores.dim() == 2 else 0
    _lib.call("dkd_frame_fuse_csr_detail", _p(q), _p(table), _p(clip_scores), _p(key_clip), _p(vid_ptr), _p(q_list),
              _p(slot), Nv, P, D, w_clip, w_frame, w_branch, int(accumulate), _p(cand_scores), dense_ld, _p(payload),
              payload.shape[-1], c0, _stream())
    return cand_scores


def scatter_fuse_detail(a, b, wa, wb, arg_a, arg_b, csr, cand_scores, payload):
    vid_ptr, q_list, slot = csr
    _chk(a, torch.float32, "a")
    _chk(arg_a, torch.int32, "arg_a")
    _chk(payload, torch.int32, "payload")
    _lib.call("dkd_scatter_fuse_detail", _p(a), _p(b), wa, wb, _p(arg_a), _p(arg_b), _p(slot), _p(vid_ptr),
              vid_ptr.numel() - 1, a.numel(), _p(cand_scores), _p(payload), payload.shape[-1], _stream())
    return cand_scores


def scatter_fuse(a, b, wa, wb, csr, cand_scores):
    vid_ptr, q_list, slot = csr
    _chk(a, torch.float32, "a")
    _lib.call("dkd_scatter_fuse", _p(a), _p(b), wa, wb, _p(slot), _p(vid_ptr), vid_ptr.numel() - 1, a.numel(),
              _p(cand_scores), _stream())
    return cand_scores


def row_inv_norms(x, eps=1e-12):
    _chk(x, torch.float32, "x")
    D = x.shape[-1]
    rows = x.numel() // D
    out = torch.empty((rows,), dtype=torch.float32, device=x.device)
    _lib.call("dkd_row_inv_norms", _p(x), rows, D, eps, _p(out), _stream())
    return out


TRAIN_SIM_TENSOR_CORES = True


def train_sim_fwd_tc(q, x, mask=None, labels=None, want_unnorm=True):
    M, D = q.shape
    N, L, _ = x.shape
    qn, _ = normalize_rows(q)
    xn, _ = normalize_rows(x)
    xn = xn.view(N, L, D)
    max_n, arg_n = score_max_exact(qn, pack_rows(xn), L, mask)
    max_u = arg_u = curve = None
    if want_unnorm:
        max_u, arg_u = score_max_exact(q, pack_rows(x), L, mask)
    if labels is not None:
        curve = torch.empty((M, L), dtype=torch.float32, device=q.device)
        _lib.call("dkd_train_curve", _p(qn), _p(xn), _p(mask), _p(labels), M, L, D, _p(curve), _stream())
    return max_n, arg_n, max_u, arg_u, curve


def train_sim_fwd(q, x, rq, rx, mask=None, labels=None, want_unnorm=True):
    _chk(q, torch.float32, "q")
    _chk(x, torch.float32, "x")
    M, D = q.shape
    N, L, _ = x.shape
    if mask is not None:
        _chk(mask, torch.uint8, "mask")
    if labels is not None:
        _chk(labels, torch.int32, "labels")
    if TRAIN_SIM_TENSOR_CORES and D % 32 == 0 and D <= 512 and L <= 128 and M > 0 and N > 0:
        return train_sim_fwd_tc(q, x, mask, labels, want_unnorm)
    dev = q.device
    max_n = torch.empty((M, N), dtype=torch.float32, device=dev)
    arg_n = torch.empty((M, N), dtype=torch.int32, device=dev)
    max_u = torch.empty((M, N), dtype=torch.float32, device=dev) if want_unnorm else None
    arg_u = torch.empty((M, N), dtype=torch.int32, device=dev) if want_unnorm else None
    curve = torch.empty((M, L), dtype=torch.float32, device=dev) if labels is not None else None
    _lib.call("dkd_train_sim_fwd", _p(q), _p(x), _p(rq), _p(rx), _p(mask), _p(labels), M, N, L, D, _p(max_n),
              _p(arg_n), _p(max_u), _p(arg_u), _p(curve), _stream())
    return max_n, arg_n, max_u, arg_u, curve


def train_sim_bwd(q, x, rq, rx, mask, labels, max_n, arg_n, arg_u, curve, g_n, g_u, g_c, want_q=True, want_x=True):
    M, D = q.shape
    N, L, _ = x.shape
    for name, g in (("g_max_n", g_n), ("g_max_u", g_u), ("g_curve", g_c)):
        if g is not None:
            _chk(g, torch.float32, name)
    gq = torch.empty_like(q) if want_q else None
    gx = torch.empty_like(x) if want_x else None
    _lib.call("dkd_train_sim_bwd", _p(q), _p(x), _p(rq), _p(rx), _p(mask), _p(labels), M, N, L, D, _p(max_n),
              _p(arg_n), _p(arg_u), _p(curve), _p(g_n), _p(g_u), _p(g_c), _p(gq), _p(gx), _stream())
    return gq, gx


def kl_curve_loss(pred, target, lens, temp):
    _chk(pred, torch.float32, "pred")
    _chk(target, torch.float32, "target")
    _chk(lens, torch.int32, "lens")
    M, L = pred.shape
    loss = torch.empty((M,), dtype=torch.float32, device=pred.device)
    dpred = torch.empty((M, L), dtype=torch.float32, device=pred.device)
    _lib.call("dkd_kl_curve_loss", _p(pred), _p(target), _p(lens), M, L, float(temp), _p(loss), _p(dpred), _stream())
    return loss, dpred


def train_losses(s_n, s_u, sims, labels, t2v_draw, v2t_pick, margin, soft, alpha, belta):
    _chk(s_n, torch.float32, "s_n")
    _chk(s_u, torch.float32, "s_u")
    if soft:
        _chk(sims, torch.float32, "sims")
    for name, t in (("labels", labels), ("t2v_draw", t2v_draw), ("v2t_pick", v2t_pick)):
        _chk(t, torch.int32, name)
    M, N = s_n.shape
    dev = s_n.device
    terms = torch.empty((2,), dtype=torch.float32, device=dev)
    g_n = torch.empty((M, N), dtype=torch.float32, device=dev)
    g_u = torch.empty((M, N), dtype=torch.float32, device=dev)
    ws = torch.empty((int(_lib.load().dkd_train_losses_workspace_floats(M, N)),), dtype=torch.float32, device=dev)
    _lib.call("dkd_train_losses", _p(s_n), _p(s_u), _p(sims) if soft else None, _p(labels), _p(t2v_draw), _p(v2t_pick),
              M, N, float(margin), int(bool(soft)), float(alpha), float(belta), _p(terms), _p(g_n), _p(g_u), _p(ws),
              _stream())
    return terms, g_n, g_u


def pack_weight(w):
    _chk(w, torch.float32, "weight")
    N, K = w.shape
    nbytes = int(_lib.load().dkd_weight_planes_bytes(N, K))
    if nbytes < 0:
        raise _lib.DkdError("pack_weight: K must be a multiple of 32")
    planes = torch.empty((nbytes // 4,), dtype=torch.float32, device=w.device)
    _lib.call("dkd_pack_weight_tf32", _p(w), N, K, _p(planes), _stream())
    return planes


def linear_exact(x, w_planes, N, bias=None, relu=False, row_scale_shift=None, out=None):
    _chk(x, torch.float32, "x")
    _chk(w_planes, torch.float32, "w_planes")
    M, K = x.shape
    if bias is not None:
        _chk(bias, torch.float32, "bias")
    if row_scale_shift is not None:
        _chk(row_scale_shift, torch.float32, "row_scale_shift")
    if out is None:
        out = torch.empty((M, N), dtype=torch.float32, device=x.device)
    _chk(out, torch.float32, "out")
    _lib.call("dkd_linear_exact", _p(x), M, K, _p(w_planes), N, _p(bias), int(bool(relu)), _p(row_scale_shift), _p(out),
              out.shape[1], _stream())
    return out


def row_stats(x, eps=1e-5):
    _chk(x, torch.float32, "x")
    D = x.shape[-1]
    rows = x.numel() // D
    out = torch.empty((rows, 2), dtype=torch.float32, device=x.device)
    _lib.call("dkd_row_stats", _p(x), rows, D, float(eps), _p(out), _stream())
    return out


def layernorm_rows(x, gamma, beta, eps=1e-5, residual=None, pos=None, L=0):
    rows, D = x.shape
    for name, t in (("x", x), ("residual", residual)):
        if t is not None and (not t.is_cuda or t.dtype != torch.float32 or t.stride(1) != 1):
            raise _lib.DkdError(f"layernorm_rows: {name} must be an fp32 CUDA matrix with unit column stride")
    _chk(gamma, torch.float32, "gamma")
    _chk(beta, torch.float32, "beta")
    if pos is not None:
        _chk(pos, torch.float32, "pos")
    out = torch.empty((rows, D), dtype=torch.float32, device=x.device)
    _lib.call("dkd_layernorm_rows", _p(x), x.stride(0), rows, D, _p(gamma), _p(beta), float(eps), _p(residual),
              residual.stride(0) if residual is not None else 0, _p(pos), int(L), _p(out), _stream())
    return out


def mha_small(qkv, Nv, L, heads, dh, mask=None, q_off=0, k_off=None, v_off=None):
    _chk(qkv, torch.float32, "qkv")
    H = heads * dh
    k_off = H if k_off is None else k_off
    v_off = 2 * H if v_off is None else v_off
    if mask is not None:
        _chk(mask, torch.uint8, "mask")
    out = torch.empty((Nv * L, H), dtype=torch.float32, device=qkv.device)
    _lib.call("dkd_mha_small", _p(qkv), qkv.shape[1], q_off, k_off, v_off, _p(mask), Nv, L, heads, dh,
              1.0 / float(dh) ** 0.5, _p(out), H, _stream())
    return out
```

### include/dkd_b200.h

```cpp
#ifndef DKD_B200_H_
#define DKD_B200_H_

#include <stdint.h>

#ifdef __cplusplus
extern "C" {
#endif

#define DKD_OK 0
#define DKD_ERR_ARG (-1)
#define DKD_ERR_SHAPE (-2)
#define DKD_ERR_ALIGN (-3)
#define DKD_ERR_DRIVER (-4)
#define DKD_ERR_WORKSPACE (-5)

#define DKD_MASKED_SCORE (-1e10f)

int dkd_version(void);
const char* dkd_error_string(int code);

int dkd_normalize_rows(const float* x, int64_t rows, int32_t D, float eps, float* out_f32,
                       uint16_t* out_bf16, uint16_t* out_f16, int64_t rows_out_pad, void* stream);

int dkd_downsample_clips(const float* frames, const int32_t* lengths, int32_t Nv, int32_t L,
                         int32_t D, int32_t T, float* clips, void* stream);

int dkd_build_proposals(const float* clips, int32_t Nv, int32_t T, int32_t D,
                        uint16_t* prop_bf16, float* prop_scale, float* prop_f32, void* stream);

int dkd_score_max_f32(const float* qn, int32_t M, const float* xn, int32_t Nv, int32_t R,
                      int32_t D, const uint8_t* mask, float* out_max, int32_t* out_arg,
                      int64_t ld_out, float* out_rows, const int32_t* vid_ptr,
                      const int32_t* q_list, void* stream);

int64_t dkd_row_planes_bytes(int32_t Nv, int32_t R, int32_t D);
int dkd_pack_rows_tf32(const float* xn, int32_t Nv, int32_t R, int32_t D, float* planes, void* stream);
int dkd_score_max_exact(const float* qn, int32_t M, const float* row_planes, int32_t Nv, int32_t R,
                        int32_t D, const uint8_t* mask, float* out_max, int32_t* out_arg, int64_t ld_out,
                        const int32_t* vid_ptr, const int32_t* q_list, void* stream);
int64_t dkd_clip_planes_bytes(int32_t Nv, int32_t D);
int dkd_pack_clips_tf32(const float* clips, int32_t Nv, int32_t T, int32_t D, float* planes, void* stream);
int dkd_clip_score_f32(const float* qn, int32_t M, const float* clip_planes, const float* prop_scale,
                       int32_t Nv, int32_t T, int32_t D, float* out_max, int32_t* out_arg,
                       int64_t ld_out, const int32_t* vid_ptr, const int32_t* vid_cnt,
                       const int32_t* q_list, const int32_t* out_slot, const int32_t* known_key,
                       int64_t known_ld, void* stream);

int dkd_score_max_bf16(const uint16_t* q_bf16, int32_t M, int32_t Mpad, const uint16_t* x_bf16,
                       int32_t Nv, int32_t R, int32_t D, const uint8_t* mask, float* out_max,
                       int32_t* out_arg, float* out_gap, int64_t ld_out, uint32_t* out_flags, float tau,
                       void* stream);

int dkd_score_max_f16(const uint16_t* q_f16, int32_t M, int32_t Mpad, const uint16_t* x_f16,
                      int32_t Nv, int32_t R, int32_t D, const uint8_t* mask, float* out_max,
                      int32_t* out_arg, float* out_gap, int64_t ld_out, uint32_t* out_flags, float tau,
                      void* stream);
int dkd_build_proposals_f16(const float* clips, int32_t Nv, int32_t T, int32_t D, uint16_t* prop_f16,
                            float* prop_scale, void* stream);

int dkd_score_max_bf16_lists(const uint16_t* q, int32_t M, int32_t Mpad, const uint16_t* x, int32_t Nv, int32_t R,
                             int32_t D, const uint8_t* mask, float* out_max, int32_t* out_arg, int64_t ld_out,
                             float tau, int32_t* flag_cnt, int32_t* flag_list, int64_t flag_cap,
                             int32_t f16_operands, void* stream);
int dkd_clip_score_list(const float* qn, int32_t M, const float* clip_planes, const float* prop_scale, int32_t Nv,
                        int32_t T, int32_t D, float* out_max, int32_t* out_arg, int64_t ld_out,
                        const int32_t* vid_cnt, const int32_t* q_list, int64_t list_stride, void* stream);

int dkd_select_flagged(const uint32_t* flags, int32_t M, int32_t Nv, int64_t ld, int64_t cap, int32_t* cursor,
                       int32_t* vid_begin, int32_t* vid_cnt, int32_t* q_list, int32_t* slot, void* stream);

int dkd_select_pairs_csr(const float* gap, int32_t M, int32_t Nv, int64_t ld, float tau, int64_t cap,
                         int32_t* counts, int32_t* vid_ptr, int32_t* q_list, int32_t* slot, void* stream);

int dkd_key_clip_dots(const float* key, const float* clips, int32_t Nv, int32_t L, int32_t T,
                      int32_t D, float* E, void* stream);
int dkd_frame_attn_table(const float* E, const float* val, const int32_t* lengths, int32_t Nv,
                         int32_t L, int32_t T, int32_t D, float* table_f32, uint16_t* table_f16,
                         void* stream);

int dkd_frame_fuse(const void* q, const void* table, int32_t is_f16, const float* clip_scores,
                   const int32_t* key_clip, int32_t M, int32_t Nv, int32_t P, int32_t D,
                   int64_t ld, float w_clip, float w_frame, float w_branch, int32_t accumulate,
                   float* out_frame, float* fused, void* stream);

int dkd_fuse_scores(const float* a, const float* b, float wa, float wb, float* out, int64_t n,
                    void* stream);

int dkd_topk(const float* scores, int32_t M, int32_t Nv, int64_t ld, int32_t K, int32_t id_base,
             float* out_scores, int32_t* out_ids, void* stream);

int dkd_select_topk(const float* scores, int32_t M, int32_t Nv, int64_t ld, int32_t K, int32_t id_base,
                    int32_t* out_ids, float* out_kth, void* stream);

int dkd_merge_topk(const float* scores, const int32_t* ids, int32_t G, int32_t M, int32_t K,
                   float* out_scores, int32_t* out_ids, void* stream);
int dkd_merge_topk_payload(const float* scores, const int32_t* ids, const uint32_t* payload, int32_t G, int32_t M,
                           int32_t K, int32_t C, float* out_scores, int32_t* out_ids, uint32_t* out_payload,
                           void* stream);

int dkd_rank_of_gt(const float* scores, int32_t M, int32_t Nv, int64_t ld, const int32_t* gt_ptr,
                   const int32_t* gt_ids, int32_t* out_rank, void* stream);

int dkd_candidates_to_csr(const int32_t* cand_ids, int32_t M, int32_t K, int32_t Nv,
                          int32_t id_base, int32_t* counts, int32_t* vid_ptr, int32_t* q_list,
                          int32_t* slot, void* stream);
int dkd_frame_fuse_csr(const float* q, const float* table, const float* clip_scores,
                       const int32_t* key_clip, const int32_t* vid_ptr, const int32_t* q_list,
                       const int32_t* slot, int32_t Nv, int32_t P, int32_t D, float w_clip,
                       float w_frame, float w_branch, int32_t accumulate, float* cand_scores,
                       int64_t dense_ld, void* stream);
int dkd_frame_fuse_csr_detail(const float* q, const float* table, const float* clip_scores,
                              const int32_t* key_clip, const int32_t* vid_ptr, const int32_t* q_list,
                              const int32_t* slot, int32_t Nv, int32_t P, int32_t D, float w_clip,
                              float w_frame, float w_branch, int32_t accumulate, float* cand_scores,
                              int64_t dense_ld, uint32_t* payload, int32_t C, int32_t c0, void* stream);
int dkd_scatter_fuse(const float* a, const float* b, float wa, float wb, const int32_t* slot,
                     const int32_t* vid_ptr, int32_t Nv, int64_t max_entries, float* out, void* stream);
int dkd_scatter_fuse_detail(const float* a, const float* b, float wa, float wb, const int32_t* arg_a,
                            const int32_t* arg_b, const int32_t* slot, const int32_t* vid_ptr, int32_t Nv,
                            int64_t max_entries, float* out, uint32_t* payload, int32_t C, void* stream);
int dkd_sort_candidates(const float* cand_scores, const int32_t* cand_ids, int32_t M, int32_t K,
                        int32_t K_out, float* out_scores, int32_t* out_ids, void* stream);
int dkd_sort_candidates_payload(const float* cand_scores, const int32_t* cand_ids, const uint32_t* payload,
                                int32_t M, int32_t K, int32_t K_out, int32_t C, float* out_scores, int32_t* out_ids,
                                uint32_t* out_payload, void* stream);

int dkd_row_inv_norms(const float* x, int64_t rows, int32_t D, float eps, float* out, void* stream);
int dkd_train_curve(const float* qn, const float* xn, const uint8_t* mask, const int32_t* labels, int32_t M, int32_t L,
                    int32_t D, float* curve, void* stream);
int dkd_train_sim_fwd(const float* q, const float* x, const float* rq, const float* rx, const uint8_t* mask,
                      const int32_t* labels, int32_t M, int32_t N, int32_t L, int32_t D, float* max_n,
                      int32_t* arg_n, float* max_u, int32_t* arg_u, float* curve, void* stream);
int dkd_train_sim_bwd(const float* q, const float* x, const float* rq, const float* rx, const uint8_t* mask,
                      const int32_t* labels, int32_t M, int32_t N, int32_t L, int32_t D, const float* max_n,
                      const int32_t* arg_n, const int32_t* arg_u, const float* curve, const float* g_max_n,
                      const float* g_max_u, const float* g_curve, float* grad_q, float* grad_x, void* stream);
int dkd_kl_curve_loss(const float* pred, const float* target, const int32_t* lens, int32_t M, int32_t L,
                      float temp, float* loss, float* dpred, void* stream);

int64_t dkd_train_losses_workspace_floats(int32_t M, int32_t N);
int dkd_train_losses(const float* s_n, const float* s_u, const float* sims, const int32_t* labels,
                     const int32_t* t2v_draw, const int32_t* v2t_pick, int32_t M, int32_t N, float margin,
                     int32_t soft, float alpha, float belta, float* out_terms, float* g_n, float* g_u,
                     float* workspace, void* stream);

int64_t dkd_weight_planes_bytes(int32_t N, int32_t K);
int dkd_pack_weight_tf32(const float* w, int32_t N, int32_t K, float* planes, void* stream);
int dkd_linear_exact(const float* x, int64_t M, int32_t K, const float* w_planes, int32_t N, const float* bias,
                     int32_t relu, const float* row_scale_shift, float* out, int64_t ld_out, void* stream);
int dkd_row_stats(const float* x, int64_t rows, int32_t D, float eps, float* scale_shift, void* stream);
int dkd_layernorm_rows(const float* x, int64_t x_ld, int64_t rows, int32_t D, const float* gamma, const float* beta,
                       float eps, const float* residual, int64_t res_ld, const float* pos, int32_t L, float* out,
                       void* stream);
int dkd_mha_small(const float* qkv, int64_t ld, int32_t q_off, int32_t k_off, int32_t v_off, const uint8_t* mask,
                  int32_t Nv, int32_t L, int32_t heads, int32_t dh, float scale, float* out, int64_t out_ld,
                  void* stream);

#ifdef __cplusplus
}
#endif
#endif
```

Measured before the change: 1.180 billion.

## Pre-split query TF32 planes once and restructure mode-0 clip scoring pipeline

Adds a pack kernel that splits normalized queries into TF32 hi/lo planes once per query set, so the clip-score stager warps copy both planes and skip the per-tile split_tf32 work. The mode-0 kernel drops the resident-B path and always streams clip planes through a configurable B-stage ring. It also splits the scan warps into two groups that each take one TMEM buffer, so two tiles' epilogues can run at once. In exchange the staging copy traffic for queries doubles, extra shared memory and barriers are used, and the legacy non-CSR call path passes a null plane pointer.

After: 1.148 billion (median of 6 runs). 2.7% lower.

```diff
diff --git a/dl-dkd_b200/_lib.py b/dl-dkd_b200/_lib.py
--- a/dl-dkd_b200/_lib.py
+++ b/dl-dkd_b200/_lib.py
@@ -22,7 +22,8 @@
     "dkd_score_max_exact": [_P, _I, _P, _I, _I, _I, _P, _P, _P, _L, _P, _P, _P],
     "dkd_clip_planes_bytes": [_I, _I],
     "dkd_pack_clips_tf32": [_P, _I, _I, _I, _P, _P],
-    "dkd_clip_score_f32": [_P, _I, _P, _P, _I, _I, _I, _P, _P, _L, _P, _P, _P, _P, _P, _L, _P],
+    "dkd_pack_queries_tf32": [_P, _I, _I, _P, _P],
+    "dkd_clip_score_f32": [_P, _P, _I, _P, _P, _I, _I, _I, _P, _P, _L, _P, _P, _P, _P, _P, _L, _P],
     "dkd_score_max_bf16": [_P, _I, _I, _P, _I, _I, _I, _P, _P, _P, _P, _L, _P, _F, _P],
     "dkd_score_max_f16": [_P, _I, _I, _P, _I, _I, _I, _P, _P, _P, _P, _L, _P, _F, _P],
     "dkd_score_max_bf16_lists": [_P, _I, _I, _P, _I, _I, _I, _P, _P, _P, _L, _F, _P, _P, _L, _I, _P],
diff --git a/dl-dkd_b200/csrc/dkd_exact_umma.cu b/dl-dkd_b200/csrc/dkd_exact_umma.cu
--- a/dl-dkd_b200/csrc/dkd_exact_umma.cu
+++ b/dl-dkd_b200/csrc/dkd_exact_umma.cu
@@ -13,17 +13,25 @@
 constexpr int kXThreads = (kXLoadWarp + 1) * 32;
 constexpr int kXMaxAStages = 7;
 constexpr int kXBStages = 3;
+#ifndef DKD_X_BST0
+#define DKD_X_BST0 3
+#endif
+#ifndef DKD_X_RING0
+#define DKD_X_RING0 4
+#endif
+constexpr int kXBStages0 = DKD_X_BST0;
+constexpr int kXBStagesMax = kXBStages0 > kXBStages ? kXBStages0 : kXBStages;
 constexpr uint32_t kXBPlane = 32 * 128;
 constexpr int kXTmemCols = 512;
 constexpr uint32_t kXRowPitch = 128;
 constexpr uint32_t kXSlotBytes = 32 * kXRowPitch;
 constexpr uint32_t kXScanScratch = 32 * kXRows * 4;
+constexpr int kXRing0 = DKD_X_RING0;
 
 struct ExactParams {
   const float* q; int M;
   const float* planes; const float* scale;
   int Nv, T, D;
-  int b_bufs;
   int R, Npad;
   const uint8_t* mask;
   float* out_max; int32_t* out_arg; int64_t ld_out;
@@ -44,20 +52,13 @@
 #ifndef DKD_X_KNOWN
 #define DKD_X_KNOWN 1
 #endif
-#ifndef DKD_X_STREAM_B0
-#define DKD_X_STREAM_B0 0
-#endif
-#ifndef DKD_X_RING0
-#define DKD_X_RING0 5
-#endif
-constexpr bool kXStreamB0 = DKD_X_STREAM_B0 != 0;
 constexpr int kXListScan = DKD_X_LIST_SCAN;
 constexpr int kXKnown = DKD_X_KNOWN;
 constexpr bool kXTwoPhaseList = kXListScan != 0 || kXKnown != 0;
 
 struct __align__(8) ExactCtl {
   uint64_t a_full[kXMaxAStages], a_empty[kXMaxAStages];
-  uint64_t b_full[kXBStages], b_empty[kXBStages];
+  uint64_t b_full[kXBStagesMax], b_empty[kXBStagesMax];
   uint64_t tmem_full[2], tmem_empty[2];
   uint32_t tmem_base;
 };
@@ -134,26 +135,27 @@
 exact_umma_kernel(const ExactParams p) {
   constexpr int kDW = kMode == 0 ? 32 : 128;
   constexpr int kScaleBufs = kMode == 2 ? kXGroup : 2;
-  constexpr int kStageSets = kMode == 2 ? 1 : 2;
-  constexpr int kScanGroups = (kMode == 0 && kXTwoPhaseList) ? 1 : 0;
-  constexpr bool kResB = kMode == 0 && !kXStreamB0;
+  constexpr int kStageSets = (kMode == 0 || kMode == 2) ? 1 : 2;
+  constexpr int kScanGroups = (kMode == 0 && kXTwoPhaseList) ? 2 : 0;
+  constexpr uint32_t kPitch = kMode == 0 ? 2 * kXRowPitch : kXRowPitch;
+  constexpr uint32_t kSlot = 32 * kPitch;
+  constexpr int kBSt = kMode == 0 ? kXBStages0 : kXBStages;
   constexpr uint32_t kXACol0 = 2 * kDW;
   constexpr int kXStages = (kXTmemCols - 2 * kDW) / 64;
   extern __shared__ __align__(1024) uint8_t smem_raw_x[];
   __shared__ __align__(16) float s_scale[kScaleBufs][32 * 32];
   uint8_t* smem = reinterpret_cast<uint8_t*>((reinterpret_cast<uintptr_t>(smem_raw_x) + 1023) & ~(uintptr_t)1023);
   const int num_kb = p.D / kXKB;
-  const uint32_t b_buf_bytes = kResB ? (uint32_t)num_kb * 2u * kXBPlane : 2u * (uint32_t)p.Npad * 128u;
+  const uint32_t b_buf_bytes = 2u * (uint32_t)p.Npad * 128u;
   uint8_t* sB = smem;
-  uint8_t* sS = sB + (size_t)(kResB ? p.b_bufs : kXBStages) * b_buf_bytes;
-  float* sD = reinterpret_cast<float*>(sS + (size_t)(4 * kStageSets) * kXRing * kXSlotBytes);
+  uint8_t* sS = sB + (size_t)kBSt * b_buf_bytes;
+  float* sD = reinterpret_cast<float*>(sS + (size_t)(4 * kStageSets) * kXRing * kSlot);
   ExactCtl* ctl = reinterpret_cast<ExactCtl*>(reinterpret_cast<uint8_t*>(sD) + (size_t)kScanGroups * kXScanScratch);
   const int warp = threadIdx.x >> 5, lane = threadIdx.x & 31;
-  const uint32_t b_bufs = (uint32_t)p.b_bufs;
 
   if (threadIdx.x == 0) {
     for (int i = 0; i < kXStages; ++i) { mbar_init(&ctl->a_full[i], kXStagers); mbar_init(&ctl->a_empty[i], 1); }
-    for (int i = 0; i < kXBStages; ++i) { mbar_init(&ctl->b_full[i], 1); mbar_init(&ctl->b_empty[i], 1); }
+    for (int i = 0; i < kXBStagesMax; ++i) { mbar_init(&ctl->b_full[i], 1); mbar_init(&ctl->b_empty[i], 1); }
     for (int i = 0; i < 2; ++i) {
       mbar_init(&ctl->tmem_full[i], 1);
       mbar_init(&ctl->tmem_empty[i], kXScanWarps);
@@ -175,8 +177,9 @@
     const int cl_row = lane >> 3, cl_chunk = lane & 7;
     const uint32_t a_lane = tmem_base + ((uint32_t)(quarter * 32) << 16) + kXACol0;
     const int sw = warp - kXScanWarps;
-    const uint32_t ring0 = smem_u32(sS) + (uint32_t)sw * kXRing * kXSlotBytes;
-    const uint8_t* ring_ptr = sS + (size_t)sw * kXRing * kXSlotBytes;
+    const uint32_t ring0 = smem_u32(sS) + (uint32_t)sw * kXRing * kSlot;
+    const uint8_t* ring_ptr = sS + (size_t)sw * kXRing * kSlot;
+    const int64_t q_ld = kMode == 0 ? 2 * (int64_t)p.D : (int64_t)p.D;
     uint32_t it_base = 0;
     for (int n = blockIdx.x; n < p.Nv; n += gridDim.x) {
       int e0, count, row_base = 0;
@@ -204,25 +207,36 @@
             const int r = tile * kXRows + quarter * 32 + 4 * i + cl_row;
             const bool live = r < count;
             const int64_t qrow = live ? (p.q_list ? (int64_t)p.q_list[e0 + r] : (int64_t)(row_base + r)) : 0;
-            src_cached[i] = p.q + qrow * p.D + 4 * cl_chunk;
+            src_cached[i] = p.q + qrow * q_ld + 4 * cl_chunk;
             live_mask |= (live ? 1u : 0u) << i;
           }
         }
-        const uint32_t dst = ring0 + (uint32_t)slot * kXSlotBytes + (uint32_t)cl_row * kXRowPitch +
+        const uint32_t dst = ring0 + (uint32_t)slot * kSlot + (uint32_t)cl_row * kPitch +
                              (uint32_t)((cl_chunk ^ ((cl_row & 1) << 2)) << 4);
 #pragma unroll
-        for (int i = 0; i < 8; ++i)
-          cp_async16(dst + (uint32_t)(4 * i) * kXRowPitch, src_cached[i] + kb * kXKB, ((live_mask >> i) & 1u) ? 16u : 0u);
+        for (int i = 0; i < 8; ++i) {
+          const uint32_t bytes = ((live_mask >> i) & 1u) ? 16u : 0u;
+          if constexpr (kMode == 0) {
+            cp_async16(dst + (uint32_t)(4 * i) * kPitch, src_cached[i] + 2 * kb * kXKB, bytes);
+            cp_async16(dst + (uint32_t)(4 * i) * kPitch + kXRowPitch, src_cached[i] + 2 * kb * kXKB + kXKB, bytes);
+          } else {
+            cp_async16(dst + (uint32_t)(4 * i) * kPitch, src_cached[i] + kb * kXKB, bytes);
+          }
+        }
       };
       auto store = [&](int j, int slot_i) {
-        const uint8_t* slot = ring_ptr + (size_t)slot_i * kXSlotBytes;
-        float4 v[8];
-#pragma unroll
-        for (int hu = 0; hu < 4; ++hu)
-#pragma unroll
-          for (int c = 0; c < 2; ++c)
-            v[2 * hu + c] = *reinterpret_cast<const float4*>(
-                slot + (16 * (hu >> 1) + g + 8 * (hu & 1)) * kXRowPitch + (((4 * c + t) ^ ((g & 1) << 2)) << 4));
+        constexpr int kPlanes = kMode == 0 ? 2 : 1;
+        const uint8_t* slot = ring_ptr + (size_t)slot_i * kSlot;
+        float4 v[8 * kPlanes];
+#pragma unroll
+        for (int pl = 0; pl < kPlanes; ++pl)
+#pragma unroll
+          for (int hu = 0; hu < 4; ++hu)
+#pragma unroll
+            for (int c = 0; c < 2; ++c)
+              v[8 * pl + 2 * hu + c] = *reinterpret_cast<const float4*>(
+                  slot + (16 * (hu >> 1) + g + 8 * (hu & 1)) * kPitch + pl * kXRowPitch +
+                  (((4 * c + t) ^ ((g & 1) << 2)) << 4));
         if (kMode == 4) {
           if (p.row_ss) {
             const int tile_j = j / num_kb;
@@ -257,10 +271,18 @@
 #pragma unroll
             for (int c = 0; c < 2; ++c) {
               const float4 x = v[2 * (2 * h + u) + c];
-              split_tf32(x.x, rh[4 * (2 * c) + 2 * u + 0], rl[4 * (2 * c) + 2 * u + 0]);
-              split_tf32(x.y, rh[4 * (2 * c) + 2 * u + 1], rl[4 * (2 * c) + 2 * u + 1]);
-              split_tf32(x.z, rh[4 * (2 * c + 1) + 2 * u + 0], rl[4 * (2 * c + 1) + 2 * u + 0]);
-              split_tf32(x.w, rh[4 * (2 * c + 1) + 2 * u + 1], rl[4 * (2 * c + 1) + 2 * u + 1]);
+              if constexpr (kMode == 0) {
+                const float4 y = v[8 + 2 * (2 * h + u) + c];
+                rh[4 * (2 * c) + 2 * u + 0] = __float_as_uint(x.x); rl[4 * (2 * c) + 2 * u + 0] = __float_as_uint(y.x);
+                rh[4 * (2 * c) + 2 * u + 1] = __float_as_uint(x.y); rl[4 * (2 * c) + 2 * u + 1] = __float_as_uint(y.y);
+                rh[4 * (2 * c + 1) + 2 * u + 0] = __float_as_uint(x.z); rl[4 * (2 * c + 1) + 2 * u + 0] = __float_as_uint(y.z);
+                rh[4 * (2 * c + 1) + 2 * u + 1] = __float_as_uint(x.w); rl[4 * (2 * c + 1) + 2 * u + 1] = __float_as_uint(y.w);
+              } else {
+                split_tf32(x.x, rh[4 * (2 * c) + 2 * u + 0], rl[4 * (2 * c) + 2 * u + 0]);
+                split_tf32(x.y, rh[4 * (2 * c) + 2 * u + 1], rl[4 * (2 * c) + 2 * u + 1]);
+                split_tf32(x.z, rh[4 * (2 * c + 1) + 2 * u + 0], rl[4 * (2 * c + 1) + 2 * u + 0]);
+                split_tf32(x.w, rh[4 * (2 * c + 1) + 2 * u + 1], rl[4 * (2 * c + 1) + 2 * u + 1]);
+              }
             }
           const uint32_t ta = a_lane + ((uint32_t)(16 * h) << 16) + stage * 64u;
           tmem_st_16x256b_x4(ta, rh);
@@ -289,7 +311,7 @@
     }
   } else if (warp == kXLoadWarp) {
     if (lane == 0) {
-      uint32_t vi = 0, itb = 0;
+      uint32_t itb = 0;
       for (int n = blockIdx.x; n < p.Nv; n += gridDim.x) {
         int e0, count;
         if (kMode == 2) {
@@ -317,47 +339,30 @@
         if (kMode == 4) { int r0_; item_range_linear(p, n, vid, r0_, count); }
         else video_range(p, n, e0, count);
         if (count <= 0) continue;
-        if (kResB) {
-          const uint32_t bb = vi % b_bufs;
-          mbar_wait_backoff(&ctl->b_empty[bb], ((vi / b_bufs) & 1u) ^ 1u, 5 * p.wait_ns);
-          ++vi;
-          mbar_expect_tx(&ctl->b_full[bb], b_buf_bytes);
-          const uint8_t* src = reinterpret_cast<const uint8_t*>(p.planes) + (size_t)n * b_buf_bytes;
-          for (int kb = 0; kb < num_kb; ++kb)
-            bulk_load(sB + (size_t)bb * b_buf_bytes + (size_t)kb * 2 * kXBPlane, src + (size_t)kb * 2 * kXBPlane,
-                      2 * kXBPlane, &ctl->b_full[bb]);
-        } else {
-          const uint8_t* src = reinterpret_cast<const uint8_t*>(p.planes) + (size_t)vid * num_kb * b_buf_bytes;
-          for (int t0 = 0; t0 < count; t0 += kXRows) {
-            for (int kb = 0; kb < num_kb; ++kb, ++itb) {
-              const uint32_t bs = itb % (uint32_t)kXBStages;
-              mbar_wait_backoff(&ctl->b_empty[bs], ((itb / (uint32_t)kXBStages) & 1u) ^ 1u, 5 * p.wait_ns);
-              mbar_expect_tx(&ctl->b_full[bs], b_buf_bytes);
-              bulk_load(sB + (size_t)bs * b_buf_bytes, src + (size_t)kb * b_buf_bytes, b_buf_bytes, &ctl->b_full[bs]);
-            }
+        const uint8_t* src = reinterpret_cast<const uint8_t*>(p.planes) + (size_t)vid * num_kb * b_buf_bytes;
+        for (int t0 = 0; t0 < count; t0 += kXRows) {
+          for (int kb = 0; kb < num_kb; ++kb, ++itb) {
+            const uint32_t bs = itb % (uint32_t)kBSt;
+            mbar_wait_backoff(&ctl->b_empty[bs], ((itb / (uint32_t)kBSt) & 1u) ^ 1u, 5 * p.wait_ns);
+            mbar_expect_tx(&ctl->b_full[bs], b_buf_bytes);
+            bulk_load(sB + (size_t)bs * b_buf_bytes, src + (size_t)kb * b_buf_bytes, b_buf_bytes, &ctl->b_full[bs]);
           }
         }
       }
     }
   } else if (warp == kXMmaWarp) {
-    const int nb = kMode == 0 ? 32 : p.Npad;
+    const int nb = p.Npad;
     const uint32_t idesc = make_idesc_tf32(nb, kXRows);
     const uint32_t b_plane = (uint32_t)nb * 128u;
     const bool elected = elect_one();
     const uint64_t bdesc0 = make_smem_desc(smem_u32(sB));
-    uint32_t it = 0, vi = 0, tc = 0, itb = 0;
+    uint32_t it = 0, tc = 0, itb = 0;
     for (int n = blockIdx.x; n < p.Nv; n += gridDim.x) {
       int e0, count;
       if (kMode == 2) { int g_, r_; item_range(p, n, g_, r_, count); e0 = 0; }
       else if (kMode == 4) { int g_, r_; item_range_linear(p, n, g_, r_, count); e0 = 0; }
       else video_range(p, n, e0, count);
       if (count <= 0) continue;
-      uint32_t bb = 0;
-      if (kResB) {
-        bb = vi % b_bufs;
-        mbar_wait_backoff(&ctl->b_full[bb], (vi / b_bufs) & 1u, p.wait_ns);
-        ++vi;
-      }
       for (int t0 = 0; t0 < count; t0 += kXRows, ++tc) {
         const uint32_t buf = tc & 1u;
         mbar_wait_backoff(&ctl->tmem_empty[buf], ((tc >> 1) & 1u) ^ 1u, p.wait_ns);
@@ -366,19 +371,15 @@
         for (int kb = 0; kb < num_kb; ++kb, ++it) {
           const uint32_t stage = it % (uint32_t)kXStages;
           const uint32_t phase = (it / (uint32_t)kXStages) & 1u;
-          uint32_t bs = 0;
-          if (!kResB) {
-            bs = itb % (uint32_t)kXBStages;
-            mbar_wait_backoff(&ctl->b_full[bs], (itb / (uint32_t)kXBStages) & 1u, p.wait_ns);
-            ++itb;
-          }
+          const uint32_t bs = itb % (uint32_t)kBSt;
+          mbar_wait_backoff(&ctl->b_full[bs], (itb / (uint32_t)kBSt) & 1u, p.wait_ns);
+          ++itb;
           mbar_wait_backoff(&ctl->a_full[stage], phase, p.wait_ns);
           tc_fence_after();
           if (elected) {
             const uint32_t a_hi = tmem_base + kXACol0 + stage * 64u;
             const uint32_t a_lo = a_hi + 32u;
-            const uint64_t b_hi = kResB ? bdesc0 + (uint64_t)((bb * b_buf_bytes + (uint32_t)kb * 2u * b_plane) >> 4)
-                                             : bdesc0 + (uint64_t)((bs * b_buf_bytes) >> 4);
+            const uint64_t b_hi = bdesc0 + (uint64_t)((bs * b_buf_bytes) >> 4);
             const uint64_t b_lo = b_hi + (uint64_t)(b_plane >> 4);
 #pragma unroll
             for (int k = 0; k < 4; ++k) {
@@ -387,15 +388,11 @@
               umma_tf32_ts(d_tmem, a_hi + 8 * k, b_hi + 2 * k, idesc, 1u);
             }
             umma_commit(&ctl->a_empty[stage]);
-            if (!kResB) umma_commit(&ctl->b_empty[bs]);
+            umma_commit(&ctl->b_empty[bs]);
           }
           __syncwarp();
         }
         if (elected) umma_commit(&ctl->tmem_full[buf]);
-        __syncwarp();
-      }
-      if (kResB) {
-        if (elected) umma_commit(&ctl->b_empty[bb]);
         __syncwarp();
       }
     }
@@ -457,15 +454,17 @@
     }
   } else if constexpr (kMode == 0) {
     const int T = p.T, P = T * (T + 1) / 2;
-    const int quarter = warp;
+    const int quarter = warp & 3;
+    const uint32_t part = warp >= 2 * kXScanWarps ? 1u : 0u;
     const int stid = threadIdx.x;
+    float* dcol = sD + part * (kXScanScratch / 4) + quarter * 32 + lane;
     uint32_t tc = 0, vi = 0;
     for (int n = blockIdx.x; n < p.Nv; n += gridDim.x) {
       int e0, count;
       video_range(p, n, e0, count);
       if (count <= 0) continue;
       float* sc = s_scale[vi & 1u];
-      {
+      if (part == 0) {
         const float* gsc = p.scale + (int64_t)n * P;
         const int s_ = stid & 31;
         int base = 0;
@@ -474,10 +473,11 @@
           base += T - w + 1;
         }
       }
-      asm volatile("bar.sync 1, %0;" ::"n"(kXScanWarps * 32) : "memory");
+      asm volatile("bar.sync 1, %0;" ::"n"(2 * kXScanWarps * 32) : "memory");
       ++vi;
       for (int t0 = 0; t0 < count; t0 += kXRows, ++tc) {
         const uint32_t buf = tc & 1u;
+        if (buf != part) continue;
         mbar_wait(&ctl->tmem_full[buf], (tc >> 1) & 1u);
         tc_fence_after();
         uint32_t raw[32];
@@ -493,9 +493,8 @@
         int bi0;
         const int r = t0 + quarter * 32 + lane;
         if constexpr (kT32 && kXTwoPhaseList) {
-          float* dcol = sD + quarter * 32 + lane;
           if (kXKnown != 0 && p.known_key) {
-            const int qi = r < count ? (p.q_list ? p.q_list[e0 + r] : r) : 0;
+            const int qi = r < count ? p.q_list[e0 + r] : 0;
             const int key = r < count ? __ldg(p.known_key + (int64_t)qi * p.known_ld + n) : 0;
             window_scan_known<kXKnown == 2>(d, sc, dcol, kXRows, key, bv0, bi0);
           } else if (kXListScan != 0) {
@@ -508,8 +507,7 @@
         }
         if (r < count) {
           const int64_t o = p.out_slot ? (int64_t)p.out_slot[e0 + r]
-                            : (p.list_stride > 0 ? (int64_t)p.q_list[e0 + r] * p.ld_out + n
-                                                 : (p.vid_ptr ? (int64_t)(e0 + r) : (int64_t)r * p.ld_out + n));
+                            : (p.list_stride > 0 ? (int64_t)p.q_list[e0 + r] * p.ld_out + n : (int64_t)(e0 + r));
           p.out_max[o] = bv0;
           if (p.out_arg) p.out_arg[o] = bi0;
         }
@@ -631,9 +629,34 @@
   }
 }
 
+__global__ void pack_queries_tf32_kernel(const float4* __restrict__ qn, int64_t n4, int D, float4* __restrict__ planes) {
+  const int64_t i = (int64_t)blockIdx.x * blockDim.x + threadIdx.x;
+  if (i >= n4) return;
+  const float4 x = qn[i];
+  const int64_t m = i / (D / 4);
+  const int f4 = (int)(i - m * (D / 4));
+  uint4 h, l;
+  split_tf32(x.x, h.x, l.x); split_tf32(x.y, h.y, l.y); split_tf32(x.z, h.z, l.z); split_tf32(x.w, h.w, l.w);
+  float4* dst = planes + (m * (D / kXKB) + (f4 >> 3)) * 16 + (f4 & 7);
+  dst[0] = *reinterpret_cast<const float4*>(&h);
+  dst[8] = *reinterpret_cast<const float4*>(&l);
+}
+
 }
 
 using namespace dkd;
+
+extern "C" int dkd_pack_queries_tf32(const float* qn, int32_t M, int32_t D, float* q_planes, void* stream) {
+  if (!qn || !q_planes || M < 0) return DKD_ERR_ARG;
+  if (D <= 0 || D % kXKB != 0 || D > 512) return DKD_ERR_SHAPE;
+  if ((reinterpret_cast<uintptr_t>(qn) | reinterpret_cast<uintptr_t>(q_planes)) & 15) return DKD_ERR_ALIGN;
+  if (M == 0) return DKD_OK;
+  const int64_t n4 = (int64_t)M * (D / 4);
+  pack_queries_tf32_kernel<<<(unsigned)((n4 + 255) / 256), 256, 0, (cudaStream_t)stream>>>(
+      reinterpret_cast<const float4*>(qn), n4, D, reinterpret_cast<float4*>(q_planes));
+  DKD_LAUNCH_CHECK();
+  return DKD_OK;
+}
 
 static int row_pad(int R, int clip_mode) { return clip_mode ? 32 : ((R + 15) / 16) * 16; }
 
@@ -670,24 +693,14 @@
   DKD_CUDA_TRY(cudaGetDevice(&dev));
   DKD_CUDA_TRY(cudaDeviceGetAttribute(&sms, cudaDevAttrMultiProcessorCount, dev));
   DKD_CUDA_TRY(cudaDeviceGetAttribute(&max_smem, cudaDevAttrMaxSharedMemoryPerBlockOptin, dev));
-  const int num_kb = D / kXKB;
-  const bool stream0 = mode == 0 && kXStreamB0;
-  const int ring = stream0 ? DKD_X_RING0 : ((mode == 0 || mode == 2) && D > 448 ? 2 : 3);
-  const int ring_warps = mode == 2 ? 4 : kXStageWarps;
-  const int scan_groups = (mode == 0 && kXTwoPhaseList) ? 1 : 0;
+  const int ring = mode == 0 ? kXRing0 : (mode == 2 && D > 448 ? 2 : 3);
+  const int ring_warps = (mode == 0 || mode == 2) ? 4 : kXStageWarps;
+  const size_t slot = mode == 0 ? 2 * kXSlotBytes : kXSlotBytes;
+  const int scan_groups = (mode == 0 && kXTwoPhaseList) ? 2 : 0;
   const size_t fixed = sizeof(ExactCtl) + 1024 + 128 + 16384  +
-                       (size_t)ring_warps * ring * kXSlotBytes + (size_t)scan_groups * kXScanScratch;
-  size_t b_total;
-  if (mode == 0 && !stream0) {
-    const size_t b_buf = (size_t)num_kb * 2 * kXBPlane;
-    if ((size_t)max_smem < fixed + b_buf) return DKD_ERR_SHAPE;
-    p.b_bufs = ((size_t)max_smem >= fixed + 2 * b_buf) ? 2 : 1;
-    b_total = (size_t)p.b_bufs * b_buf;
-  } else {
-    p.b_bufs = kXBStages;
-    b_total = (size_t)kXBStages * 2 * p.Npad * 128;
-    if ((size_t)max_smem < fixed + b_total) return DKD_ERR_SHAPE;
-  }
+                       (size_t)ring_warps * ring * slot + (size_t)scan_groups * kXScanScratch;
+  const size_t b_total = (size_t)(mode == 0 ? kXBStages0 : kXBStages) * 2 * p.Npad * 128;
+  if ((size_t)max_smem < fixed + b_total) return DKD_ERR_SHAPE;
   const size_t smem = fixed - 16384 + b_total;
   const int grid = p.Nv < sms ? p.Nv : sms;
   auto launch = [&](auto kern) -> int {
@@ -696,11 +709,8 @@
     return DKD_OK;
   };
   int rc;
-  if (mode == 0 && stream0) {
-    rc = (T == 32) ? launch(exact_umma_kernel<0, true, DKD_X_RING0>) : launch(exact_umma_kernel<0, false, DKD_X_RING0>);
-  } else if (mode == 0) {
-    if (ring == 3) rc = (T == 32) ? launch(exact_umma_kernel<0, true, 3>) : launch(exact_umma_kernel<0, false, 3>);
-    else rc = (T == 32) ? launch(exact_umma_kernel<0, true, 2>) : launch(exact_umma_kernel<0, false, 2>);
+  if (mode == 0) {
+    rc = (T == 32) ? launch(exact_umma_kernel<0, true, kXRing0>) : launch(exact_umma_kernel<0, false, kXRing0>);
   } else if (mode == 2) {
     if (ring == 3) rc = (T == 32) ? launch(exact_umma_kernel<2, true, 3>) : launch(exact_umma_kernel<2, false, 3>);
     else rc = (T == 32) ? launch(exact_umma_kernel<2, true, 2>) : launch(exact_umma_kernel<2, false, 2>);
@@ -731,27 +741,28 @@
   return launch_exact(1, p, D, 0, (cudaStream_t)stream);
 }
 
-extern "C" int dkd_clip_score_f32(const float* qn, int32_t M, const float* clip_planes, const float* prop_scale,
-                                  int32_t Nv, int32_t T, int32_t D, float* out_max, int32_t* out_arg,
-                                  int64_t ld_out, const int32_t* vid_ptr, const int32_t* vid_cnt,
+extern "C" int dkd_clip_score_f32(const float* qn, const float* q_planes, int32_t M, const float* clip_planes,
+                                  const float* prop_scale, int32_t Nv, int32_t T, int32_t D, float* out_max,
+                                  int32_t* out_arg, int64_t ld_out, const int32_t* vid_ptr, const int32_t* vid_cnt,
                                   const int32_t* q_list, const int32_t* out_slot, const int32_t* known_key,
                                   int64_t known_ld, void* stream) {
-  if (!qn || !clip_planes || !prop_scale || !out_max || M < 0 || Nv < 0) return DKD_ERR_ARG;
+  const float* q = vid_ptr ? q_planes : qn;
+  if (!q || !clip_planes || !prop_scale || !out_max || M < 0 || Nv < 0) return DKD_ERR_ARG;
   if ((vid_ptr == nullptr) != (q_list == nullptr)) return DKD_ERR_ARG;
   if ((out_slot || vid_cnt) && !vid_ptr) return DKD_ERR_ARG;
   if (known_key && (!vid_ptr || known_ld < Nv || T != 32)) return DKD_ERR_ARG;
   if (T <= 0 || T > 32 || D <= 0 || D % kXKB != 0 || D > 512) return DKD_ERR_SHAPE;
   if (!vid_ptr && ld_out < Nv) return DKD_ERR_ARG;
-  if ((reinterpret_cast<uintptr_t>(qn) | reinterpret_cast<uintptr_t>(clip_planes) | reinterpret_cast<uintptr_t>(prop_scale)) & 15)
+  if ((reinterpret_cast<uintptr_t>(q) | reinterpret_cast<uintptr_t>(clip_planes) | reinterpret_cast<uintptr_t>(prop_scale)) & 15)
     return DKD_ERR_ALIGN;
   if (M == 0 || Nv == 0) return DKD_OK;
   ExactParams p{};
-  p.q = qn; p.M = M; p.planes = clip_planes; p.scale = prop_scale;
+  p.q = q; p.M = M; p.planes = clip_planes; p.scale = prop_scale;
   p.Nv = Nv; p.T = T; p.D = D; p.R = T; p.Npad = 32; p.mask = nullptr;
   p.out_max = out_max; p.out_arg = out_arg; p.ld_out = ld_out;
   p.vid_ptr = vid_ptr; p.vid_cnt = vid_cnt; p.q_list = q_list; p.out_slot = out_slot;
   p.known_key = known_key; p.known_ld = known_ld;
-  if (!vid_ptr && Nv >= kXGroup) {
+  if (!vid_ptr) {
     const int groups = (Nv + kXGroup - 1) / kXGroup;
     const int tiles = (M + kXRows - 1) / kXRows;
     int sms = 148, dev = 0;
@@ -809,17 +820,18 @@
   return launch_exact(4, p, K, 0, (cudaStream_t)stream);
 }
 
-extern "C" int dkd_clip_score_list(const float* qn, int32_t M, const float* clip_planes, const float* prop_scale,
+extern "C" int dkd_clip_score_list(const float* q_planes, int32_t M, const float* clip_planes, const float* prop_scale,
                                    int32_t Nv, int32_t T, int32_t D, float* out_max, int32_t* out_arg, int64_t ld_out,
                                    const int32_t* vid_cnt, const int32_t* q_list, int64_t list_stride, void* stream) {
-  if (!qn || !clip_planes || !prop_scale || !out_max || !vid_cnt || !q_list || M < 0 || Nv < 0) return DKD_ERR_ARG;
+  if (!q_planes || !clip_planes || !prop_scale || !out_max || !vid_cnt || !q_list || M < 0 || Nv < 0) return DKD_ERR_ARG;
   if (list_stride <= 0 || ld_out < Nv || (int64_t)Nv * list_stride > 0x7fffffffLL) return DKD_ERR_ARG;
   if (T <= 0 || T > 32 || D <= 0 || D % kXKB != 0 || D > 512) return DKD_ERR_SHAPE;
-  if ((reinterpret_cast<uintptr_t>(qn) | reinterpret_cast<uintptr_t>(clip_planes) | reinterpret_cast<uintptr_t>(prop_scale)) & 15)
+  if ((reinterpret_cast<uintptr_t>(q_planes) | reinterpret_cast<uintptr_t>(clip_planes) |
+       reinterpret_cast<uintptr_t>(prop_scale)) & 15)
     return DKD_ERR_ALIGN;
   if (M == 0 || Nv == 0) return DKD_OK;
   ExactParams p{};
-  p.q = qn; p.M = M; p.planes = clip_planes; p.scale = prop_scale;
+  p.q = q_planes; p.M = M; p.planes = clip_planes; p.scale = prop_scale;
   p.Nv = Nv; p.T = T; p.D = D; p.R = T; p.Npad = 32; p.mask = nullptr;
   p.out_max = out_max; p.out_arg = out_arg; p.ld_out = ld_out;
   p.vid_ptr = nullptr; p.vid_cnt = vid_cnt; p.q_list = q_list; p.out_slot = nullptr; p.list_stride = list_stride;
diff --git a/dl-dkd_b200/engine.py b/dl-dkd_b200/engine.py
--- a/dl-dkd_b200/engine.py
+++ b/dl-dkd_b200/engine.py
@@ -122,6 +122,7 @@
     qn: List[torch.Tensor]
     qb: List[torch.Tensor]
     qh: List[torch.Tensor]
+    qp: Optional[List[torch.Tensor]] = None
 
 
 _PAD_WORDS = {}
@@ -187,7 +188,7 @@
 def prepare_queries(q_by_branch, want_bf16=True) -> PreparedQueries:
     M = q_by_branch[0].shape[0]
     Mpad = ops.round_up(max(M, 1), 256)
-    qn, qb, qh = [], [], []
+    qn, qb, qh, qp = [], [], [], []
     if M == 0:
         return PreparedQueries(M=0, Mpad=Mpad, qn=[q.float() for q in q_by_branch], qb=[None] * len(q_by_branch),
                                qh=[None] * len(q_by_branch))
@@ -197,7 +198,12 @@
         qn.append(f[:M])
         qb.append(b)
         qh.append(h)
-    return PreparedQueries(M=M, Mpad=Mpad, qn=qn, qb=qb, qh=qh)
+        qp.append(ops.pack_queries(qn[-1]))
+    return PreparedQueries(M=M, Mpad=Mpad, qn=qn, qb=qb, qh=qh, qp=qp)
+
+
+def _q_planes(pq: PreparedQueries, bi):
+    return pq.qp[bi] if pq.qp is not None else None
 
 
 def _branch_weights(nb):
@@ -250,7 +256,8 @@
                 prop = bd.prop_b
             if tau > 0:
                 s_clip, k_clip, cnt, lst = ops.score_max_bf16_lists(qb, pq.M, prop, pc.Nv, pc.Pg, tau, mask=pc.prop_mask)
-                ops.clip_score_list(qn, bd.clip_planes, bd.prop_scale, cnt, lst, s_clip, k_clip)
+                ops.clip_score_list(qn, bd.clip_planes, bd.prop_scale, cnt, lst, s_clip, k_clip,
+                                    q_planes=_q_planes(pq, bi))
             else:
                 s_clip, k_clip = ops.score_max_bf16(qb, pq.M, prop, pc.Nv, pc.Pg, mask=pc.prop_mask)
             q, tab = qh, bd.table_h
@@ -374,7 +381,7 @@
                 cs, ck = per[bi]["clip"], per[bi]["key_clip"]
             else:
                 cs, ck = ops.clip_score_f32(qn, bd.clip_planes, bd.prop_scale, csr=csr[:2],
-                                            known_key=per[bi]["key_clip"])
+                                            known_key=per[bi]["key_clip"], q_planes=_q_planes(pq, bi))
             wb = wbs[bi] if nb == 2 else 1.0
             if return_detail:
                 ops.frame_fuse_csr_detail(qn, bd.table_f, cs, ck, csr, w_clip, w_frame, wb, cand_scores, bi > 0,
diff --git a/dl-dkd_b200/eval.py b/dl-dkd_b200/eval.py
--- a/dl-dkd_b200/eval.py
+++ b/dl-dkd_b200/eval.py
@@ -134,7 +134,8 @@
                 sub = engine.PreparedCorpus(Nv=pc.Nv, L=pc.L, D=pc.D, T=pc.T, id_base=pc.id_base, mask_u8=pc.mask_u8,
                                             lengths=pc.lengths, branches=[pc.branches[bi]], heads=pc.heads,
                                             Lg=pc.Lg, mask_g=pc.mask_g, Pg=pc.Pg, prop_mask=pc.prop_mask)
-                subq = engine.PreparedQueries(M=pq.M, Mpad=pq.Mpad, qn=[pq.qn[bi]], qb=[pq.qb[bi]], qh=[pq.qh[bi]])
+                subq = engine.PreparedQueries(M=pq.M, Mpad=pq.Mpad, qn=[pq.qn[bi]], qb=[pq.qb[bi]], qh=[pq.qh[bi]],
+                                              qp=None if pq.qp is None else [pq.qp[bi]])
                 f, _ = engine.score_two_scale_head(sub, subq, precision, model.clip_scale_w, model.frame_scale_w)
                 outs[bi].append(f)
     inher = torch.cat(outs[0], dim=0).cpu().numpy().copy()
diff --git a/dl-dkd_b200/ops.py b/dl-dkd_b200/ops.py
--- a/dl-dkd_b200/ops.py
+++ b/dl-dkd_b200/ops.py
@@ -157,7 +157,26 @@
     return planes
 
 
-def clip_score_f32(qn, clips, prop_scale, csr=None, scatter=None, known_key=None):
+def pack_queries(qn):
+    _chk(qn, torch.float32, "qn")
+    M, D = qn.shape
+    if D % 32:
+        raise _lib.DkdError("pack_queries: D must be a multiple of 32")
+    qp = torch.empty((M, D // 32, 2, 32), dtype=torch.float32, device=qn.device)
+    _lib.call("dkd_pack_queries_tf32", _p(qn), M, D, _p(qp), _stream())
+    return qp
+
+
+def _query_planes(qn, q_planes):
+    if q_planes is None:
+        return pack_queries(qn)
+    _chk(q_planes, torch.float32, "q_planes")
+    if q_planes.shape != (qn.shape[0], qn.shape[1] // 32, 2, 32):
+        raise _lib.DkdError("q_planes is not pack_queries(qn)")
+    return q_planes
+
+
+def clip_score_f32(qn, clips, prop_scale, csr=None, scatter=None, known_key=None, q_planes=None):
     _chk(qn, torch.float32, "qn")
     _chk(prop_scale, torch.float32, "prop_scale")
     planes = clips if clips.dim() == 5 else pack_clips(clips)
@@ -171,9 +190,10 @@
     if csr is None:
         om = torch.empty((M, Nv), dtype=torch.float32, device=dev)
         oa = torch.empty((M, Nv), dtype=torch.int32, device=dev)
-        _lib.call("dkd_clip_score_f32", _p(qn), M, _p(planes), _p(prop_scale), Nv, T, D, _p(om), _p(oa), Nv,
+        _lib.call("dkd_clip_score_f32", _p(qn), None, M, _p(planes), _p(prop_scale), Nv, T, D, _p(om), _p(oa), Nv,
                   None, None, None, None, None, 0, _stream())
         return om, oa
+    q_planes = _query_planes(qn, q_planes)
     vid_ptr, q_list = csr[0], csr[1]
     vid_cnt = csr[2] if len(csr) > 2 else None
     if scatter is not None:
@@ -189,7 +209,7 @@
         _chk(known_key, torch.int32, "known_key")
         if T != 32 or known_key.shape != (M, Nv):
             known_key = None
-    _lib.call("dkd_clip_score_f32", _p(qn), M, _p(planes), _p(prop_scale), Nv, T, D, _p(om), _p(oa), 0,
+    _lib.call("dkd_clip_score_f32", None, _p(q_planes), M, _p(planes), _p(prop_scale), Nv, T, D, _p(om), _p(oa), 0,
               _p(vid_ptr), _p(vid_cnt), _p(q_list), _p(slot), _p(known_key), Nv if known_key is not None else 0, _stream())
     return om, oa
 
@@ -238,8 +258,9 @@
     return om, oa, cnt, lst
 
 
-def clip_score_list(qn, planes, prop_scale, cnt, lst, out_max, out_arg):
+def clip_score_list(qn, planes, prop_scale, cnt, lst, out_max, out_arg, q_planes=None):
     _chk(qn, torch.float32, "qn")
+    q_planes = _query_planes(qn, q_planes)
     _chk(planes, torch.float32, "clip_planes")
     _chk(prop_scale, torch.float32, "prop_scale")
     _chk(cnt, torch.int32, "flag_cnt")
@@ -249,7 +270,7 @@
     M, D = qn.shape
     Nv, P = prop_scale.shape
     T = int(round(((8 * P + 1) ** 0.5 - 1) / 2))
-    _lib.call("dkd_clip_score_list", _p(qn), M, _p(planes), _p(prop_scale), Nv, T, D, _p(out_max), _p(out_arg),
+    _lib.call("dkd_clip_score_list", _p(q_planes), M, _p(planes), _p(prop_scale), Nv, T, D, _p(out_max), _p(out_arg),
               out_max.shape[1], _p(cnt), _p(lst), lst.shape[1], _stream())
     return out_max, out_arg
 
diff --git a/include/dkd_b200.h b/include/dkd_b200.h
--- a/include/dkd_b200.h
+++ b/include/dkd_b200.h
@@ -40,8 +40,9 @@
                         const int32_t* vid_ptr, const int32_t* q_list, void* stream);
 int64_t dkd_clip_planes_bytes(int32_t Nv, int32_t D);
 int dkd_pack_clips_tf32(const float* clips, int32_t Nv, int32_t T, int32_t D, float* planes, void* stream);
-int dkd_clip_score_f32(const float* qn, int32_t M, const float* clip_planes, const float* prop_scale,
-                       int32_t Nv, int32_t T, int32_t D, float* out_max, int32_t* out_arg,
+int dkd_pack_queries_tf32(const float* qn, int32_t M, int32_t D, float* q_planes, void* stream);
+int dkd_clip_score_f32(const float* qn, const float* q_planes, int32_t M, const float* clip_planes,
+                       const float* prop_scale, int32_t Nv, int32_t T, int32_t D, float* out_max, int32_t* out_arg,
                        int64_t ld_out, const int32_t* vid_ptr, const int32_t* vid_cnt,
                        const int32_t* q_list, const int32_t* out_slot, const int32_t* known_key,
                        int64_t known_ld, void* stream);
@@ -62,7 +63,7 @@
                              int32_t D, const uint8_t* mask, float* out_max, int32_t* out_arg, int64_t ld_out,
                              float tau, int32_t* flag_cnt, int32_t* flag_list, int64_t flag_cap,
                              int32_t f16_operands, void* stream);
-int dkd_clip_score_list(const float* qn, int32_t M, const float* clip_planes, const float* prop_scale, int32_t Nv,
+int dkd_clip_score_list(const float* q_planes, int32_t M, const float* clip_planes, const float* prop_scale, int32_t Nv,
                         int32_t T, int32_t D, float* out_max, int32_t* out_arg, int64_t ld_out,
                         const int32_t* vid_cnt, const int32_t* q_list, int64_t list_stride, void* stream);
 
```
